# Xharlie/BtcDet

Hardware: AMD Instinct MI355X
Metric: scenes/s fwd+bwd KITTI-Car bs=2/GPU (BtcDet hot path) (higher is better)
Workload: dtype f32

## Files before the change

btcdet_amd/csrc/btc_common.h:

```cpp
#pragma once
#include <hip/hip_runtime.h>
#include <stdint.h>
#include <stdio.h>

#include "../../include/btcdet_hip.h"

#define BTC_EMPTY_KEY (-1)
#define BTC_EMPTY_IDX 0x7F7F7F7F

void btc_set_error(const char* fmt, ...);

#define BTC_CHECK_ARG(cond, ...)            \
  do {                                      \
    if (!(cond)) {                          \
      btc_set_error(__VA_ARGS__);           \
      return BTC_EINVAL;                    \
    }                                       \
  } while (0)

#define BTC_HIP(call)                                                             \
  do {                                                                            \
    hipError_t e_ = (call);                                                       \
    if (e_ != hipSuccess) {                                                       \
      btc_set_error("%s failed: %s (%s:%d)", #call, hipGetErrorString(e_), __FILE__, __LINE__); \
      return BTC_ELAUNCH;                                                         \
    }                                                                             \
  } while (0)

#define BTC_LAUNCH_CHECK()                                                        \
  do {                                                                            \
    hipError_t e_ = hipGetLastError();                                            \
    if (e_ != hipSuccess) {                                                       \
      btc_set_error("kernel launch failed: %s (%s:%d)", hipGetErrorString(e_), __FILE__, __LINE__); \
      return BTC_ELAUNCH;                                                         \
    }                                                                             \
  } while (0)

#if defined(__HIP_DEVICE_COMPILE__) && !defined(__gfx950__)
#error "the fence-free last-arriver protocol (btc_ticket_take) is derived for gfx950's sc1 write-through stores only"
#endif
#if defined(__HIPCC__)
template <class T>
__device__ __forceinline__ void btc_st_agent(T* p, T v) { __hip_atomic_store(p, v, __ATOMIC_RELAXED, __HIP_MEMORY_SCOPE_AGENT); }
template <class T>
__device__ __forceinline__ T btc_ld_agent(const T* p) { return __hip_atomic_load(p, __ATOMIC_RELAXED, __HIP_MEMORY_SCOPE_AGENT); }
__device__ __forceinline__ int btc_ticket_take(int32_t* counter) {
  asm volatile("s_waitcnt vmcnt(0)" ::: "memory");
  return __hip_atomic_fetch_add(counter, 1, __ATOMIC_RELAXED, __HIP_MEMORY_SCOPE_AGENT);
}
__device__ __forceinline__ void btc_ticket_acquire() { __builtin_amdgcn_fence(__ATOMIC_ACQUIRE, "agent"); }
#endif

#define BTC_TUNE_KEYS 24
int btc_tune_get(int key);

bool btc_apply_glds_supported(int K, int Cred, int Cres);
bool btc_apply_glds_has_shape(int shape, bool bf = false);
size_t btc_apply_glds_lds_bytes(int shape, int kc, int K, bool bf, int stages = 3);
int btc_apply_glds_stages(int shape, int kc, int K, bool bf, int asked);
int btc_launch_apply_glds(bool trans_w, int shape, int kc, int xcd, bool bf, const void* feat, const float* W, const float* bias,
                          const int32_t* nbr, const int32_t* order , int n_rows, int K, int Cred, int Cres, void* out,
                          hipStream_t stream, const struct BnFuse* bn = nullptr );

int btc_apply(const char* who, int pass, int operands, const void* src, long long src_rows, const void* W, const float* bias, const int32_t* nbr,
              const int32_t* order, int n_rows, int K, int Cin, int Cout, void* dst, hipStream_t stream, const struct BnFuse* bn);

int btc_apply_bf16w(const void* src, const void* Wq, const float* bias, const int32_t* nbr, const int32_t* order, int n_rows, int K, int Cred,
                    int Cres, void* dst, hipStream_t stream, int mirror = 0, const struct BnFuse* bn = nullptr);
constexpr size_t BTC_SCRATCH_HEAD = 64 * 1024;
constexpr long long BTC_SCRATCH_TICKETS = BTC_SCRATCH_HEAD / 4;
void* btc_scratch(hipStream_t stream, size_t* bytes);
struct BnFuse;
int btc_apply_split(const float* src, const void* Ws, const float* bias, const int32_t* nbr, const int32_t* order, int n_rows, int K, int Cred,
                    int Cres, float* dst, hipStream_t stream, int mirror, const BnFuse* bn);

__host__ __device__ __forceinline__ unsigned short btc_f32_to_bf16(float f) {
  union { float f; unsigned u; } c;
  c.f = f;
  unsigned u = c.u;
  if ((u & 0x7fffffffu) > 0x7f800000u) return (unsigned short)((u >> 16) | 0x40);
  u += 0x7fffu + ((u >> 16) & 1u);
  return (unsigned short)(u >> 16);
}
__host__ __device__ __forceinline__ float btc_bf16_to_f32(unsigned short h) {
  union { float f; unsigned u; } c;
  c.u = (unsigned)h << 16;
  return c.f;
}

template <bool BF>
__device__ __forceinline__ float4 btc_ld4(const float* base, size_t i) {
  if (!BF) return *reinterpret_cast<const float4*>(base + i);
  const uint2 v = *reinterpret_cast<const uint2*>(reinterpret_cast<const unsigned short*>(base) + i);
  return make_float4(__uint_as_float(v.x << 16), __uint_as_float(v.x & 0xffff0000u), __uint_as_float(v.y << 16),
                     __uint_as_float(v.y & 0xffff0000u));
}
template <bool BF>
__device__ __forceinline__ float btc_ld1(const float* base, size_t i) {
  if (!BF) return base[i];
  return __uint_as_float((unsigned)reinterpret_cast<const unsigned short*>(base)[i] << 16);
}
template <bool BF>
__device__ __forceinline__ void btc_st4(float* base, size_t i, float a, float b, float c, float d) {
  if (!BF) {
    *reinterpret_cast<float4*>(base + i) = make_float4(a, b, c, d);
  } else {
    uint2 v;
    v.x = (unsigned)btc_f32_to_bf16(a) | ((unsigned)btc_f32_to_bf16(b) << 16);
    v.y = (unsigned)btc_f32_to_bf16(c) | ((unsigned)btc_f32_to_bf16(d) << 16);
    *reinterpret_cast<uint2*>(reinterpret_cast<unsigned short*>(base) + i) = v;
  }
}
template <bool BF>
__device__ __forceinline__ void btc_st1(float* base, size_t i, float a) {
  if (!BF) base[i] = a;
  else reinterpret_cast<unsigned short*>(base)[i] = btc_f32_to_bf16(a);
}

#ifdef __cplusplus
#include <mutex>
constexpr int BTC_MAX_DEVICES = 16;
struct BtcPerDeviceOnce {
  std::once_flag flag[BTC_MAX_DEVICES];
};
template <class F>
static inline void btc_once_per_device(BtcPerDeviceOnce& o, F&& fn) {
  int dev = 0;
  (void)hipGetDevice(&dev);
  std::call_once(o.flag[dev >= 0 && dev < BTC_MAX_DEVICES ? dev : 0], fn);
}
#endif

typedef float f32x4 __attribute__((ext_vector_type(4)));
constexpr int TM = 64;
__host__ __device__ constexpr int ldb_of(int nt) { return nt * 16 + (((nt * 16) % 32 == 0) ? 16 : 0); }

static inline int btc_cdiv(long long a, long long b) { return (int)((a + b - 1) / b); }
static inline size_t btc_align(size_t x, size_t a = 256) { return (x + a - 1) / a * a; }
static inline unsigned btc_pow2_ge(unsigned long long v) {
  unsigned long long p = 1;
  while (p < v) p <<= 1;
  return (unsigned)p;
}

struct BtcCarver {
  char* base;
  size_t off;
  explicit BtcCarver(void* p) : base((char*)p), off(0) {}
  template <typename T>
  T* take(size_t count) {
    T* r = (T*)(base + off);
    off += btc_align(count * sizeof(T));
    return r;
  }
};

size_t btc_scan_ws_bytes(long long n);
int btc_scan_exclusive_i32(const int32_t* in, int32_t* out, long long n, int32_t* total, void* ws, hipStream_t stream);

size_t btc_bytemap_bytes(long long nwords);
int btc_bytemap_to_ranked_bitmap(const unsigned char* bytemap, long long nwords, unsigned* bitmap, int32_t* prefix, int32_t* total,
                                 void* ws, hipStream_t stream);

struct BtcGeom {
  int in_shape[3];
  int out_shape[3];
  int k[3];
  int s[3];
  int p[3];
  int d[3];
  int K;
  int mode;
};

__device__ __forceinline__ unsigned btc_hash32(unsigned key) {
  key *= 2654435761u;
  key ^= key >> 15;
  return key;
}
```

btcdet_amd/csrc/conv_apply_bf16.hip:

```cpp
#include "conv_tile.h"

namespace {

__device__ unsigned short g_zero_row_b[128];

constexpr int B_STAGES = 3;

template <int WR, int WC, int NTW, int KC, bool PAIR = false>
__global__ __launch_bounds__(64 * WR * WC) void conv_apply_b(const unsigned short* __restrict__ feat, const unsigned short* __restrict__ Wq,
                                                             const float* __restrict__ bias, const int32_t* __restrict__ nbr,
                                                             const int32_t* __restrict__ order, int n_rows, int K, int Cred, int Cres,
                                                             unsigned short* __restrict__ out, int flags, const BnFuse bn) {
  extern __shared__ __attribute__((aligned(16))) char smem[];
  constexpr int NW = WR * WC, THREADS = 64 * NW;
  constexpr int TM = 16 * WR, TN = 16 * NTW * WC;
  constexpr int UPR = KC / 8;
  constexpr int RPB = (128 / (KC * 2)) < 1 ? 1 : (128 / (KC * 2));
  constexpr int A_UNITS = TM * UPR, B_UNITS = TN * UPR;
  constexpr int NAI_TOTAL = (A_UNITS + 63) / 64, NAI = (NAI_TOTAL + NW - 1) / NW;
  constexpr int NBI_TOTAL = (B_UNITS + 63) / 64, NBI = (NBI_TOTAL + NW - 1) / NW;
  constexpr int NPI = NAI + NBI;
  constexpr int A_BYTES = (TM * KC * 2 + 1023) / 1024 * 1024;
  constexpr int B_BYTES = (TN * KC * 2 + 1023) / 1024 * 1024;
  constexpr int STAGE = A_BYTES + B_BYTES;
  char* ring = smem;
  APPLY_TAIL(ring + B_STAGES * STAGE, TM, K);

  const int tid = threadIdx.x, lane = tid & 63, wave = tid >> 6;
  const int wr = wave / WC, wc = wave % WC;
  const ApplyTile tile = apply_tile_prologue<TM, THREADS>(s_nbr, s_kact, s_nact, s_row, nbr, order, n_rows, K, flags, wr);
  const int bx = tile.bx, n0 = blockIdx.y * TN, n_act = tile.n_act;
  const unsigned long long wave_act = tile.wave_act;
  static_assert(!PAIR || KC == 64, "PAIR: two 32-channel offsets per 64-channel item");
  const int n_chunks = PAIR ? 1 : Cred / KC;
  const int n_items = PAIR ? (n_act + 1) >> 1 : n_act * n_chunks;

  f32x4 acc[NTW];
#pragma unroll
  for (int nt = 0; nt < NTW; ++nt) acc[nt] = (f32x4){0.f, 0.f, 0.f, 0.f};

  int iq = 0, ir = 0, cq = 0, cr = 0;
  auto issue = [&](int st) {
    const int k = s_kact[PAIR ? 2 * iq : iq];
    const int k1 = (PAIR && 2 * iq + 1 < n_act) ? s_kact[2 * iq + 1] : -1;
    const int cc = PAIR ? 0 : ir * KC;
    if (++ir == n_chunks) { ir = 0; ++iq; }
    char* As = ring + st * STAGE;
    char* Bs = As + A_BYTES;
#pragma unroll
    for (int t = 0; t < NAI; ++t) {
      const int ai = (wave + NW * t) % NAI_TOTAL;
      const int U = ai * 64 + lane;
      if (A_UNITS % 64 == 0 || U < A_UNITS) {
        const int rloc = U / UPR;
        const int u = (U % UPR) ^ ((rloc / RPB) & (UPR - 1));
        const int ku = (PAIR && (u & 4)) ? k1 : k;
        const int nb = ku >= 0 ? s_nbr[rloc * K + ku] : -1;
        const unsigned short* src = nb >= 0 ? feat + (size_t)nb * Cred + cc + (PAIR ? (u & 3) : u) * 8 : g_zero_row_b;
        glds16(src, As + ai * 1024);
      }
    }
    const unsigned short* Wk = Wq + ((size_t)k * Cres + n0) * Cred + cc;
    const unsigned short* Wk1 = PAIR ? Wq + ((size_t)(k1 >= 0 ? k1 : k) * Cres + n0) * Cred : Wk;
#pragma unroll
    for (int t = 0; t < NBI; ++t) {
      const int bi = (wave + NW * t) % NBI_TOTAL;
      const int U = bi * 64 + lane;
      if (B_UNITS % 64 == 0 || U < B_UNITS) {
        const int c = U / UPR;
        const int u = (U % UPR) ^ ((c / RPB) & (UPR - 1));
        glds16(((PAIR && (u & 4)) ? Wk1 : Wk) + (size_t)c * Cred + (PAIR ? (u & 3) : u) * 8, Bs + bi * 1024);
      }
    }
  };

  const int arow = lane & 15, kq = lane >> 4;
  if (n_items > 0) issue(0);
  if (n_items > 1) issue(1);
  int st = 0;
  for (int item = 0; item < n_items; ++item) {
    if (item + 1 < n_items) wait_vm<NPI>();
    else wait_vm<0>();
    __builtin_amdgcn_s_barrier();
    asm volatile("" ::: "memory");
    if (item + 2 < n_items) issue(st == 0 ? 2 : st - 1);
    const int k = s_kact[PAIR ? 2 * cq : cq];
    const int k2 = (PAIR && 2 * cq + 1 < n_act) ? s_kact[2 * cq + 1] : -1;
    if (++cr == n_chunks) { cr = 0; ++cq; }
    const bool act0 = (wave_act >> k) & 1ull, act1 = PAIR && k2 >= 0 && ((wave_act >> k2) & 1ull);
    if (act0 || act1) {
      const char* A = ring + st * STAGE + (wr * 16 + arow) * (KC * 2);
      const char* B = ring + st * STAGE + A_BYTES;
      const int aswz = ((wr * 16 + arow) / RPB) & (UPR - 1);
      constexpr int STEPS = KC / 32;
      bf16x8 a[STEPS], b[STEPS][NTW];
#pragma unroll
      for (int s = 0; s < STEPS; ++s) {
        const int q = s * 4 + kq;
        a[s] = *(const bf16x8*)(A + ((q ^ aswz) * 16));
#pragma unroll
        for (int nt = 0; nt < NTW; ++nt) {
          const int col = (wc * NTW + nt) * 16 + arow;
          b[s][nt] = *(const bf16x8*)(B + col * (KC * 2) + ((q ^ ((col / RPB) & (UPR - 1))) * 16));
        }
      }
#pragma unroll
      for (int s = 0; s < STEPS; ++s) {
        if (PAIR && !(s ? act1 : act0)) continue;
#pragma unroll
        for (int nt = 0; nt < NTW; ++nt)
          acc[nt] = __builtin_amdgcn_mfma_f32_16x16x32_bf16(a[s], b[s][nt], acc[nt], 0, 0, 0);
      }
    }
    st = (st == B_STAGES - 1) ? 0 : st + 1;
  }

  float vals[NTW][4];
  bool valid[4];
  int rows[4];
#pragma unroll
  for (int r = 0; r < 4; ++r) rows[r] = s_row[wr * 16 + kq * 4 + r];
  apply_tile_epilogue<NTW>(acc, rows, n0 + wc * NTW * 16, bias, Cres, out, bn, bn.ev_mean != nullptr, vals, valid);
  if (bn.slots) {
    bn_fuse_wave<NTW>(bn, vals, valid, n0 + wc * NTW * 16, (int)((bx * WR + wr) & (bn.nslots - 1)));
    bn_fuse_finish(bn, (int*)smem, (double*)(smem + 16));
  }
}

size_t lds_bytes_b(int tm, int tn, int kc, int K) {
  const size_t a = ((size_t)tm * kc * 2 + 1023) / 1024 * 1024, b = ((size_t)tn * kc * 2 + 1023) / 1024 * 1024;
  return (size_t)B_STAGES * (a + b) + apply_tail_bytes(tm, K);
}

template <int WR, int WC, int NTW, int KC, bool PAIR = false>
int launch_b(const unsigned short* feat, const unsigned short* Wq, const float* bias, const int32_t* nbr, const int32_t* order, int n_rows, int K, int Cred,
             int Cres, unsigned short* out, int flags, hipStream_t stream, const BnFuse& bn) {
  constexpr int TM = 16 * WR, TN = 16 * NTW * WC;
  return apply_launch<conv_apply_b<WR, WC, NTW, KC, PAIR>>("conv_apply_b", dim3(btc_cdiv(n_rows, TM), Cres / TN), 64 * WR * WC, lds_bytes_b(TM, TN, KC, K),
                                                          stream, feat, Wq, bias, nbr, order, n_rows, K, Cred, Cres, out, flags, bn);
}

template <int WR, int WC, int NTW>
int launch_b_kc(int kc, const unsigned short* feat, const unsigned short* Wq, const float* bias, const int32_t* nbr, const int32_t* order, int n_rows,
                int K, int Cred, int Cres, unsigned short* out, int xcd, hipStream_t stream, const BnFuse& bn) {
  if (kc == 128) return launch_b<WR, WC, NTW, 64, true>(feat, Wq, bias, nbr, order, n_rows, K, Cred, Cres, out, xcd, stream, bn);
  if (kc == 64) return launch_b<WR, WC, NTW, 64>(feat, Wq, bias, nbr, order, n_rows, K, Cred, Cres, out, xcd, stream, bn);
  return launch_b<WR, WC, NTW, 32>(feat, Wq, bias, nbr, order, n_rows, K, Cred, Cres, out, xcd, stream, bn);
}

int apply_b(const void* feat_, const void* Wq_, const float* bias, const int32_t* nbr, const int32_t* order, int n_rows, int K, int Cred, int Cres,
            void* out_, hipStream_t stream, int mirror = 0, const BnFuse* bn_ = nullptr) {
  if (n_rows <= 0) return BTC_OK;
  const BnFuse bn = bn_ ? *bn_ : btc_bn_fuse_none();
  const unsigned short* feat = (const unsigned short*)feat_;
  const unsigned short* Wq = (const unsigned short*)Wq_;
  unsigned short* out = (unsigned short*)out_;
  int kc = (Cred % 64 == 0) ? 64 : 32;
  if (Cred == 32 && K >= 8 && btc_tune_get(BTC_TUNE_SPLIT_PAIR) != 1 && (btc_tune_get(BTC_TUNE_SPLIT_PAIR) == 2 || n_rows >= 5000)) kc = 128;
  const int xcd = apply_flags(mirror);
  if (Cres % 128 == 0) return launch_b_kc<4, 2, 4>(kc, feat, Wq, bias, nbr, order, n_rows, K, Cred, Cres, out, xcd, stream, bn);
  if (Cres % 64 == 0) {
    if (n_rows < 8192) return launch_b_kc<1, 4, 1>(kc, feat, Wq, bias, nbr, order, n_rows, K, Cred, Cres, out, xcd, stream, bn);
    return launch_b_kc<4, 2, 2>(kc, feat, Wq, bias, nbr, order, n_rows, K, Cred, Cres, out, xcd, stream, bn);
  }
  if (Cres % 32 == 0) return launch_b_kc<2, 2, 1>(kc, feat, Wq, bias, nbr, order, n_rows, K, Cred, Cres, out, xcd, stream, bn);
  return launch_b_kc<4, 1, 1>(kc, feat, Wq, bias, nbr, order, n_rows, K, Cred, Cres, out, xcd, stream, bn);
}

constexpr int BF16_MULTI_MAX = 32;
struct Bf16Table {
  const float* W[BF16_MULTI_MAX];
  unsigned short* w_b[BF16_MULTI_MAX];
  unsigned short* wt_b[BF16_MULTI_MAX];
  int K[BF16_MULTI_MAX], Cin[BF16_MULTI_MAX], Cout[BF16_MULTI_MAX], first_block[BF16_MULTI_MAX + 1];
  int n;
};

__global__ __launch_bounds__(256) void weights_to_bf16_multi(const Bf16Table t) {
  int s = 0;
  while (s + 1 < t.n && (int)blockIdx.x >= t.first_block[s + 1]) ++s;
  const long long e = (long long)((int)blockIdx.x - t.first_block[s]) * 256 + threadIdx.x;
  const int Cin = t.Cin[s], Cout = t.Cout[s];
  const long long per = (long long)Cin * Cout;
  if (e >= (long long)t.K[s] * per) return;
  const unsigned short h = btc_f32_to_bf16(t.W[s][e]);
  t.w_b[s][e] = h;
  const int k = (int)(e / per);
  const int rem = (int)(e - (long long)k * per);
  const int ci = rem / Cout, co = rem - ci * Cout;
  t.wt_b[s][(long long)k * per + (long long)co * Cin + ci] = h;
}

}

extern "C" int btc_weights_to_bf16_multi(const float* const* W, void* const* w_bf16, void* const* wt_bf16, const int32_t* K, const int32_t* Cin,
                                         const int32_t* Cout, int n, void* stream) {
  BTC_CHECK_ARG(n >= 0, "btc_weights_to_bf16_multi: bad count");
  for (int base = 0; base < n; base += BF16_MULTI_MAX) {
    Bf16Table t;
    t.n = n - base < BF16_MULTI_MAX ? n - base : BF16_MULTI_MAX;
    int blocks = 0;
    for (int i = 0; i < t.n; ++i) {
      BTC_CHECK_ARG(K[base + i] >= 1 && Cin[base + i] >= 1 && Cout[base + i] >= 1, "btc_weights_to_bf16_multi: bad sizes");
      t.W[i] = W[base + i];
      t.w_b[i] = (unsigned short*)w_bf16[base + i];
      t.wt_b[i] = (unsigned short*)wt_bf16[base + i];
      t.K[i] = K[base + i]; t.Cin[i] = Cin[base + i]; t.Cout[i] = Cout[base + i];
      t.first_block[i] = blocks;
      blocks += (int)btc_cdiv((long long)K[base + i] * Cin[base + i] * Cout[base + i], 256);
    }
    t.first_block[t.n] = blocks;
    if (blocks > 0) weights_to_bf16_multi<<<blocks, 256, 0, (hipStream_t)stream>>>(t);
    BTC_LAUNCH_CHECK();
  }
  return BTC_OK;
}

int btc_apply_bf16w(const void* src, const void* Wq, const float* bias, const int32_t* nbr, const int32_t* order, int n_rows, int K, int Cred,
                    int Cres, void* dst, hipStream_t stream, int mirror, const BnFuse* bn) {
  return apply_b(src, Wq, bias, nbr, order, n_rows, K, Cred, Cres, dst, stream, mirror, bn);
}

extern "C" int btc_conv_bf16w_supported(int K, int Cred, int Cres) { return K >= 1 && K <= 64 && Cred >= 32 && Cred % 32 == 0 && Cres % 16 == 0; }

extern "C" int btc_weights_to_bf16(const float* W, int K, int Cin, int Cout, void* w_bf16, void* wt_bf16, void* stream) {
  BTC_CHECK_ARG(K >= 1 && Cin >= 1 && Cout >= 1, "btc_weights_to_bf16: bad sizes");
  return btc_weights_to_bf16_multi(&W, &w_bf16, &wt_bf16, &K, &Cin, &Cout, 1, stream);
}
```

btcdet_amd/csrc/conv_apply_glds.hip:

```cpp
#include "conv_tile.h"

namespace {

__device__ float g_zero_row[64];

constexpr int G_STAGES_DEFAULT = 3;
constexpr int G_STAGES_MAX = 8;

__device__ __forceinline__ void transpose4(const f32x4 v, float& y0, float& y1, float& y2, float& y3) {
  unsigned x0 = __float_as_uint(v[0]), x1 = __float_as_uint(v[1]), x2 = __float_as_uint(v[2]), x3 = __float_as_uint(v[3]);
  auto a = __builtin_amdgcn_permlane32_swap(x0, x2, false, false);
  x0 = a[0]; x2 = a[1];
  auto b = __builtin_amdgcn_permlane32_swap(x1, x3, false, false);
  x1 = b[0]; x3 = b[1];
  auto c = __builtin_amdgcn_permlane16_swap(x0, x1, false, false);
  x0 = c[0]; x1 = c[1];
  auto d = __builtin_amdgcn_permlane16_swap(x2, x3, false, false);
  x2 = d[0]; x3 = d[1];
  y0 = __uint_as_float(x0); y1 = __uint_as_float(x1); y2 = __uint_as_float(x2); y3 = __uint_as_float(x3);
}

template <int WR, int WC, int NTW, bool TRANS_W, int KC, bool BF>
__global__ __launch_bounds__(64 * WR * WC) void conv_apply_g(const void* __restrict__ feat_, const float* __restrict__ W,
                                                             const float* __restrict__ bias, const int32_t* __restrict__ nbr,
                                                             const int32_t* __restrict__ order, int n_rows, int K, int Cred, int Cres,
                                                             void* __restrict__ out_, int flags, int dbg, const BnFuse bn) {
  extern __shared__ __attribute__((aligned(16))) char smem[];
  const int S = ((flags >> APPLY_STAGES_SHIFT) & 15) ? ((flags >> APPLY_STAGES_SHIFT) & 15) : G_STAGES_DEFAULT;
  constexpr int NW = WR * WC, THREADS = 64 * NW;
  constexpr int TM = 16 * WR, TN = 16 * NTW * WC, NG = NTW * WC;
  constexpr int ES = BF ? 2 : 4;
  constexpr int UPR = KC * ES / 16;
  constexpr int UPB = KC / 4;
  constexpr int RPB = (128 / (KC * ES)) < 1 ? 1 : (128 / (KC * ES));
  constexpr int A_UNITS = TM * UPR;
  constexpr int NAI_TOTAL = (A_UNITS + 63) / 64;
  constexpr int NAI = (NAI_TOTAL + NW - 1) / NW;
  constexpr int NBI_TOTAL = KC * TN / 256;
  constexpr int NBI = (NBI_TOTAL + NW - 1) / NW;
  constexpr int NPI = NAI + NBI;
  constexpr int A_BYTES = (TM * KC * ES + 1023) / 1024 * 1024;
  constexpr int STAGE = A_BYTES + KC * TN * 4;
  char* ring = smem;
  APPLY_TAIL(ring + S * STAGE, TM, K);
  const char* feat = (const char*)feat_;

  const int tid = threadIdx.x, lane = tid & 63, wave = tid >> 6;
  const int wr = wave / WC, wc = wave % WC;
  const ApplyTile tile = apply_tile_prologue<TM, THREADS>(s_nbr, s_kact, s_nact, s_row, nbr, order, n_rows, K, flags, wr);
  const int bx = tile.bx, n0 = blockIdx.y * TN, n_act = tile.n_act;
  const unsigned long long wave_act = tile.wave_act;
  const int n_chunks = Cred / KC;
  const int n_items = (dbg & 32) ? 0 : n_act * n_chunks;
  if (dbg & 16) return;

  f32x4 acc[NTW];
#pragma unroll
  for (int nt = 0; nt < NTW; ++nt) acc[nt] = (f32x4){0.f, 0.f, 0.f, 0.f};

  int iq = 0, ir = 0, cq = 0, cr = 0;
  auto issue = [&](int st) {
    const int k = s_kact[iq];
    const int cc = ir * KC;
    if (++ir == n_chunks) { ir = 0; ++iq; }
    char* As = ring + st * STAGE;
    float* Bs = (float*)(As + A_BYTES);
#pragma unroll
    for (int t = 0; t < NAI; ++t) {
      if (dbg & 8) break;
      const int ai = (wave + NW * t) % NAI_TOTAL;
      const int U = ai * 64 + lane;
      if (A_UNITS % 64 == 0 || U < A_UNITS) {
        const int rloc = U / UPR;
        const int u = (U % UPR) ^ ((rloc / RPB) & (UPR - 1));
        const int nb = s_nbr[rloc * K + k];
        const char* src = nb >= 0 ? feat + ((size_t)nb * Cred + cc) * ES + u * 16 : (const char*)g_zero_row;
        glds16(src, As + ai * 1024);
      }
    }
    const float* Wk = W + (size_t)k * Cred * Cres;
#pragma unroll
    for (int t = 0; t < NBI; ++t) {
      if (dbg & 4) break;
      const int ii = (wave + NW * t) % NBI_TOTAL;
      const int U = ii * 64 + lane;
      const float* src;
      if (!TRANS_W) {
        const int kr = U / (TN / 4), pu = U % (TN / 4);
        const int g = (NG >= 2) ? ((pu >> 2) ^ (kr & 1)) : (pu >> 2);
        src = Wk + (size_t)(cc + kr) * Cres + n0 + g * 16 + (pu & 3) * 4;
      } else {
        const int c = U / UPB, pu = U % UPB;
        const int ru = pu ^ (c & (UPB - 1));
        src = Wk + (size_t)(n0 + c) * Cred + cc + ru * 4;
      }
      glds16(src, Bs + ii * 256);
    }
  };

  const int arow = lane & 15, kq = lane >> 4;
#define WAIT_ITEMS(n) wait_vm<((n) * NPI > 63 ? 63 : (n) * NPI)>()
  for (int i = 0; i < S - 1 && i < n_items; ++i) issue(i);
  int st = 0;
  for (int item = 0; item < n_items; ++item) {
    const int left = n_items - 1 - item, fl = left < S - 2 ? left : S - 2;
    switch (fl) {
      case 0: wait_vm<0>(); break;
      case 1: WAIT_ITEMS(1); break;
      case 2: WAIT_ITEMS(2); break;
      case 3: WAIT_ITEMS(3); break;
      case 4: WAIT_ITEMS(4); break;
      case 5: WAIT_ITEMS(5); break;
      default: WAIT_ITEMS(6); break;
    }
#undef WAIT_ITEMS
    __builtin_amdgcn_s_barrier();
    asm volatile("" ::: "memory");
    if (item + S - 1 < n_items && !(dbg & 2)) issue(st == 0 ? S - 1 : st - 1);
    const int k = s_kact[cq];
    if (++cr == n_chunks) { cr = 0; ++cq; }
    if (((wave_act >> k) & 1ull) && !(dbg & 1)) {
      const char* A = ring + st * STAGE + (wr * 16 + arow) * (KC * ES);
      const float* B = (const float*)(ring + st * STAGE + A_BYTES);
      const int aswz = ((wr * 16 + arow) / RPB) & (UPR - 1);
      constexpr int Q = KC / 4;
      constexpr int G = (16 / NTW) < 1 ? 1 : ((16 / NTW) > Q ? Q : (16 / NTW));
      constexpr int NGRP = Q / G;
      float a[2][G], b[2][G][NTW];
      constexpr bool A128 = !BF && (G % 4 == 0);
      constexpr bool B128 = TRANS_W && (G % 4 == 0) && UPB >= 8 && NTW == 1;
      auto load_group = [&](int g, int buf) {
        if (A128) {
#pragma unroll
          for (int jb = 0; jb < G / 4; ++jb) {
            const int u = (g * (G / 4) + jb) * 4 + kq;
            const f32x4 v = *(const f32x4*)(A + ((u ^ aswz) * 16));
            transpose4(v, a[buf][4 * jb], a[buf][4 * jb + 1], a[buf][4 * jb + 2], a[buf][4 * jb + 3]);
          }
        }
        if (B128) {
#pragma unroll
          for (int nt = 0; nt < NTW; ++nt) {
            const float* colp = B + ((wc * NTW + nt) * 16 + arow) * KC;
#pragma unroll
            for (int jb = 0; jb < G / 4; ++jb) {
              const int u = (g * (G / 4) + jb) * 4 + kq;
              const f32x4 v = *(const f32x4*)(colp + ((u ^ (arow & (UPB - 1))) * 4));
              transpose4(v, b[buf][4 * jb][nt], b[buf][4 * jb + 1][nt], b[buf][4 * jb + 2][nt], b[buf][4 * jb + 3][nt]);
            }
          }
        }
#pragma unroll
        for (int i = 0; i < G; ++i) {
          const int q = g * G + i;
          if (A128) {
          } else if (!BF) {
            a[buf][i] = *(const float*)(A + ((q ^ aswz) * 16) + kq * 4);
          } else {
            const unsigned short h = *(const unsigned short*)(A + (((q >> 1) ^ aswz) * 16) + (((q & 1) * 4 + kq) * 2));
            a[buf][i] = __uint_as_float((unsigned)h << 16);
          }
          if (!TRANS_W) {
            const float* bp = B + (q * 4 + kq) * TN + arow;
#pragma unroll
            for (int nt = 0; nt < NTW; ++nt) {
              const int cg = wc * NTW + nt;
              b[buf][i][nt] = bp[((NG >= 2) ? (cg ^ (kq & 1)) : cg) * 16];
            }
          } else if (!B128) {
            const float* bp = B + (wc * NTW * 16 + arow) * KC + (q ^ (arow & (UPB - 1))) * 4 + kq;
#pragma unroll
            for (int nt = 0; nt < NTW; ++nt) b[buf][i][nt] = bp[nt * 16 * KC];
          }
        }
      };
      load_group(0, 0);
#pragma unroll
      for (int g = 0; g < NGRP; ++g) {
        if (g + 1 < NGRP) load_group(g + 1, (g + 1) & 1);
        __builtin_amdgcn_sched_barrier(0);
#pragma unroll
        for (int i = 0; i < G; ++i)
#pragma unroll
          for (int nt = 0; nt < NTW; ++nt)
            acc[nt] = __builtin_amdgcn_mfma_f32_16x16x4f32(a[g & 1][i], b[g & 1][i][nt], acc[nt], 0, 0, 0);
        __builtin_amdgcn_sched_barrier(0);
      }
    }
    st = (st == S - 1) ? 0 : st + 1;
  }

  float vals[NTW][4];
  bool valid[4];
  int rows[4];
#pragma unroll
  for (int r = 0; r < 4; ++r) rows[r] = s_row[wr * 16 + kq * 4 + r];
  const bool ev = !TRANS_W && bn.ev_mean != nullptr;
  typedef typename std::conditional<BF, unsigned short, float>::type OUT;
  apply_tile_epilogue<NTW>(acc, rows, n0 + wc * NTW * 16, bias, Cres, (OUT*)out_, bn, ev, vals, valid);
  if (bn.slots) {
    bn_fuse_wave<NTW>(bn, vals, valid, n0 + wc * NTW * 16, (int)((bx * WR + wr) & (bn.nslots - 1)));
    bn_fuse_finish(bn, (int*)smem, (double*)(smem + 16));
  }
}

template <int WR, int WC, int NTW, bool TRANS_W, int KC, bool BF>
int launch_g(const void* feat, const float* W, const float* bias, const int32_t* nbr, const int32_t* order, int n_rows, int K, int Cred,
             int Cres, void* out, int xcd, hipStream_t stream, const BnFuse& bn) {
  constexpr int TM = 16 * WR, TN = 16 * NTW * WC;
  const int stages = btc_apply_glds_stages(WR * 100 + WC * 10 + NTW, KC, K, BF, (xcd >> APPLY_STAGES_SHIFT) & 15);
  xcd = (xcd & (APPLY_XCD | APPLY_MIRROR)) | (stages << APPLY_STAGES_SHIFT);
  const size_t lds = btc_apply_glds_lds_bytes(WR * 100 + WC * 10 + NTW, KC, K, BF, stages);
  return apply_launch<conv_apply_g<WR, WC, NTW, TRANS_W, KC, BF>>("conv_apply_g", dim3(btc_cdiv(n_rows, TM), Cres / TN), 64 * WR * WC, lds, stream, feat, W,
                                                                  bias, nbr, order, n_rows, K, Cred, Cres, out, xcd,
                                                                  btc_tune_get(BTC_TUNE_APPLY_DEBUG), bn);
}

#define G_ARGS feat, W, bias, nbr, order, n_rows, K, Cred, Cres, out, xcd, stream, bn
#define G_PARAMS                                                                                                             \
  const void *feat, const float *W, const float *bias, const int32_t *nbr, const int32_t *order, int n_rows, int K, int Cred, int Cres, \
      void *out, int xcd, hipStream_t stream, const BnFuse &bn

template <int WR, int WC, int NTW, bool TRANS_W, bool BF>
int launch_g_kc(int kc, G_PARAMS) {
  switch (kc) {
    case 16: return launch_g<WR, WC, NTW, TRANS_W, 16, BF>(G_ARGS);
    case 32: return launch_g<WR, WC, NTW, TRANS_W, 32, BF>(G_ARGS);
    default: return launch_g<WR, WC, NTW, TRANS_W, 64, BF>(G_ARGS);
  }
}

template <bool TRANS_W>
int launch_g_shape(int wr, int wc, int ntw, int kc, bool bf, G_PARAMS) {
  const int code = wr * 100 + wc * 10 + ntw;
  switch (code) {
#define G_CASE2(WR_, WC_, NTW_)                                                      \
  case WR_ * 100 + WC_ * 10 + NTW_:                                                  \
    return bf ? launch_g_kc<WR_, WC_, NTW_, TRANS_W, true>(kc, G_ARGS) : launch_g_kc<WR_, WC_, NTW_, TRANS_W, false>(kc, G_ARGS)
#define G_CASE(WR_, WC_, NTW_)      \
  case WR_ * 100 + WC_ * 10 + NTW_: \
    if (bf) break;                  \
    return launch_g_kc<WR_, WC_, NTW_, TRANS_W, false>(kc, G_ARGS)
    G_CASE2(4, 1, 1); G_CASE(4, 1, 2); G_CASE(4, 1, 4); G_CASE(4, 1, 8);
    G_CASE(4, 2, 1); G_CASE2(4, 2, 2); G_CASE2(4, 2, 4);
    G_CASE2(2, 2, 1); G_CASE(2, 2, 2); G_CASE(2, 2, 4);
    G_CASE(2, 4, 1); G_CASE(2, 4, 2);
    G_CASE2(1, 4, 1); G_CASE(1, 4, 2);
#undef G_CASE
#undef G_CASE2
    default: break;
  }
  btc_set_error("conv_apply_g: no instance for WR=%d WC=%d NTW=%d bf16=%d", wr, wc, ntw, (int)bf);
  return BTC_EINVAL;
}

}

bool btc_apply_glds_has_shape(int shape, bool bf) {
  static const int shapes[] = {411, 412, 414, 418, 421, 422, 424, 221, 222, 224, 241, 242, 141, 142};
  static const int shapes_bf[] = {411, 422, 424, 221, 141};
  if (bf) {
    for (int v : shapes_bf)
      if (v == shape) return true;
    return false;
  }
  for (int v : shapes)
    if (v == shape) return true;
  return false;
}

size_t btc_apply_glds_lds_bytes(int shape, int kc, int K, bool bf, int stages) {
  const int tm = 16 * (shape / 100), tn = 16 * ((shape / 10) % 10) * (shape % 10);
  const size_t a_bytes = ((size_t)tm * kc * (bf ? 2 : 4) + 1023) / 1024 * 1024;
  return (size_t)(stages > 0 ? stages : G_STAGES_DEFAULT) * (a_bytes + (size_t)kc * tn * 4) + apply_tail_bytes(tm, K);
}

int btc_apply_glds_stages(int shape, int kc, int K, bool bf, int asked) {
  const int tm = 16 * (shape / 100), tn = 16 * ((shape / 10) % 10) * (shape % 10), nw = (shape / 100) * ((shape / 10) % 10);
  const size_t a_bytes = ((size_t)tm * kc * (bf ? 2 : 4) + 1023) / 1024 * 1024, stage = a_bytes + (size_t)kc * tn * 4;
  const int npi = (int)(((a_bytes / 1024) + nw - 1) / nw + ((size_t)kc * tn / 256 + nw - 1) / nw);
  int s = asked ? asked : btc_tune_get(BTC_TUNE_APPLY_STAGES);
  if (!s) {
    s = (int)((size_t)48 * 1024 / stage);
    if (s > 6) s = 6;
  }
  if (s < 3) s = 3;
  if (s > G_STAGES_MAX) s = G_STAGES_MAX;
  while (s > 3 && ((s - 2) * npi > 63 || btc_apply_glds_lds_bytes(shape, kc, K, bf, s) > 160 * 1024)) --s;
  return s;
}

bool btc_apply_glds_supported(int K, int Cred, int Cres) { return K <= 64 && Cred % 16 == 0 && Cres % 16 == 0 && Cred >= 16; }

int btc_launch_apply_glds(bool trans_w, int shape, int kc, int xcd, bool bf, const void* feat, const float* W, const float* bias,
                          const int32_t* nbr, const int32_t* order, int n_rows, int K, int Cred, int Cres, void* out, hipStream_t stream,
                          const BnFuse* bn_) {
  if (n_rows <= 0) return BTC_OK;
  const BnFuse bn = bn_ ? *bn_ : btc_bn_fuse_none();
  const int wr = shape / 100, wc = (shape / 10) % 10, ntw = shape % 10;
  BTC_CHECK_ARG(btc_apply_glds_supported(K, Cred, Cres) && wc * ntw > 0 && Cres % (16 * wc * ntw) == 0 && Cred % kc == 0 &&
                    (kc == 16 || kc == 32 || kc == 64),
                "conv_apply_g: unsupported K=%d Cred=%d Cres=%d shape=%d kc=%d", K, Cred, Cres, shape, kc);
  return trans_w ? launch_g_shape<true>(wr, wc, ntw, kc, bf, G_ARGS) : launch_g_shape<false>(wr, wc, ntw, kc, bf, G_ARGS);
}
```

btcdet_amd/csrc/conv_apply_split.hip:

```cpp
#include "conv_tile.h"

namespace {

#define BTC_RSRC_RECORDS 0xFFFFFF00u
#define BTC_RSRC_ABSENT 0xFFFFFFF0u
__device__ __forceinline__ void blds16s(__amdgpu_buffer_rsrc_t rsrc, unsigned voffset, void* l) {
  __builtin_amdgcn_raw_ptr_buffer_load_lds(rsrc, (__attribute__((address_space(3))) void*)l, 16, voffset, 0, 0, 0);
}

template <int WR, int WC, int NTW, int KC, int S_STAGES, int LW, bool PAIR = false>
__global__ __launch_bounds__(64 * (WR * WC + LW)) void conv_apply_s(const float* __restrict__ feat, const unsigned short* __restrict__ Ws,
                                                             const float* __restrict__ bias, const int32_t* __restrict__ nbr,
                                                             const int32_t* __restrict__ order, int n_rows, int K, int Cred, int Cres,
                                                             float* __restrict__ out, int flags, const BnFuse bn) {
  extern __shared__ __attribute__((aligned(16))) char smem[];
  constexpr int NW = WR * WC, THREADS = 64 * (NW + LW);
  constexpr int NLD = LW ? LW : NW;
  constexpr int TM = 16 * WR, TN = 16 * NTW * WC;
  constexpr int UPA = KC / 4, UPB = KC / 8;
  constexpr int A_UNITS = TM * UPA, B_UNITS = 3 * TN * UPB;
  static_assert(A_UNITS % 64 == 0 && B_UNITS % 64 == 0, "whole DMA instructions");
  constexpr int NAI_TOTAL = A_UNITS / 64, NAI = (NAI_TOTAL + NLD - 1) / NLD;
  constexpr int NBI_TOTAL = B_UNITS / 64, NBI = (NBI_TOTAL + NLD - 1) / NLD;
  static_assert(LW == 0 || (NAI_TOTAL % LW == 0 && NBI_TOTAL % LW == 0), "the loader waves share the pieces evenly");
  constexpr int NPI = NAI + NBI;
  constexpr int A_BYTES = TM * KC * 4, P_BYTES = TN * KC * 2;
  constexpr int STAGE = A_BYTES + 3 * P_BYTES;
  char* ring = smem;
  APPLY_TAIL(ring + S_STAGES * STAGE, TM, K);

  const int tid = threadIdx.x, lane = tid & 63, wave = tid >> 6;
  const bool computes = LW == 0 || wave < NW, loads = LW == 0 || wave >= NW;
  const int wr = computes ? wave / WC : 0, wc = wave % WC;
  const int lid = LW ? wave - NW : wave;
  const int dbg = flags >> APPLY_DEBUG_SHIFT;
  const ApplyTile tile = apply_tile_prologue<TM, THREADS>(s_nbr, s_kact, s_nact, s_row, nbr, order, n_rows, K, flags, wr);
  const int bx = tile.bx, n0 = blockIdx.y * TN;
  const unsigned long long wave_act = tile.wave_act;
  const size_t plane = (size_t)K * Cred * Cres;
  const int n_act = __builtin_amdgcn_readfirstlane(tile.n_act);
  static_assert(!PAIR || KC == 64, "PAIR: two 32-channel offsets per 64-channel item");
  const int n_chunks = PAIR ? 1 : Cred / KC;
  const int n_pairs = PAIR ? (n_act + 1) >> 1 : n_act;
  const int n_all = n_pairs * n_chunks;
  const int i0 = (int)((long long)blockIdx.z * n_all / gridDim.z);
  const int n_items = (dbg & 32) ? i0 : (int)((long long)(blockIdx.z + 1) * n_all / gridDim.z);
  out += (size_t)blockIdx.z * n_rows * Cres;

  int iq = i0 / n_chunks, ir = i0 - iq * n_chunks;
  int cq = iq, cr = ir;
  const __amdgpu_buffer_rsrc_t rfeat = __builtin_amdgcn_make_buffer_rsrc((void*)feat, 0, BTC_RSRC_RECORDS, 0x00020000);
  const int kvec = lane < n_act ? s_kact[lane] : 0;
  int nbq[NAI];
  auto load_nbq = [&]() {
    if (PAIR) {
      const int k0 = __builtin_amdgcn_readlane(kvec, (2 * iq) & 63);
      const int k1 = (2 * iq + 1 < n_act) ? __builtin_amdgcn_readlane(kvec, (2 * iq + 1) & 63) : -1;
#pragma unroll
      for (int t = 0; t < NAI; ++t) {
        const int U = ((lid + NLD * t) % NAI_TOTAL) * 64 + lane;
        const int rloc = U / UPA;
        const int u = (U % UPA) ^ ((rloc ^ (rloc >> 3)) & (UPA - 1));
        const int k = (u & 8) ? k1 : k0;
        nbq[t] = k >= 0 ? s_nbr[rloc * K + k] : -1;
      }
      return;
    }
    const int k = __builtin_amdgcn_readlane(kvec, iq);
#pragma unroll
    for (int t = 0; t < NAI; ++t) {
      const int U = ((lid + NLD * t) % NAI_TOTAL) * 64 + lane;
      nbq[t] = s_nbr[(U / UPA) * K + k];
    }
  };
  if (loads) load_nbq();
  const __amdgpu_buffer_rsrc_t rw = __builtin_amdgcn_make_buffer_rsrc((void*)Ws, 0, BTC_RSRC_RECORDS, 0x00020000);
  static_assert(NLD % 2 == 0 && (TN * UPB) % 64 == 0 && 64 % UPB == 0, "one lane offset per issuing wave");
  const int w_c = lane / UPB;
  const int w_su = (lane % UPB) ^ (((w_c >> 1) + (UPB == 8 ? 4 * (lid & 1) : 0)) & (UPB - 1));
  const unsigned w_lane = (unsigned)(w_c * Cred + (PAIR ? (w_su & 3) : w_su) * 8) * 2u;
  auto issue = [&](int st) {
    const int k = __builtin_amdgcn_readlane(kvec, PAIR ? ((2 * iq) & 63) : iq);
    const int k1 = PAIR ? ((2 * iq + 1 < n_act) ? __builtin_amdgcn_readlane(kvec, (2 * iq + 1) & 63) : k) : k;
    const unsigned w_lane_i = PAIR ? w_lane + ((w_su & 4) ? (unsigned)((size_t)(k1 - k) * Cres * Cred) * 2u : 0u) : w_lane;
    const int cc = ir * KC;
    char* As = ring + st * STAGE;
    char* Bs = As + A_BYTES;
#pragma unroll
    for (int t = 0; t < NAI; ++t) {
      if (dbg & 8) break;
      const int ai = (lid + NLD * t) % NAI_TOTAL;
      const int U = ai * 64 + lane;
      const int rloc = U / UPA;
      const int u = (U % UPA) ^ ((rloc ^ (rloc >> 3)) & (UPA - 1));
      const int nb = nbq[t];
      blds16s(rfeat, nb >= 0 ? ((unsigned)nb * (unsigned)Cred + (unsigned)(PAIR ? (u & 7) * 4 : cc + u * 4)) * 4u : BTC_RSRC_ABSENT, As + ai * 1024);
    }
    const unsigned w_item = (unsigned)(((size_t)k * Cres + n0) * Cred + (PAIR ? 0 : cc)) * 2u;
#pragma unroll
    for (int t = 0; t < NBI; ++t) {
      if (dbg & 4) break;
      const int bi = (lid + NLD * t) % NBI_TOTAL;
      const int pl = (bi * 64) / (TN * UPB), c0 = ((bi * 64) % (TN * UPB)) / UPB;
      const unsigned w_piece = (unsigned)((size_t)pl * plane + (size_t)c0 * Cred) * 2u;
      __builtin_amdgcn_raw_ptr_buffer_load_lds(rw, (__attribute__((address_space(3))) void*)(Bs + bi * 1024), 16, w_lane_i, w_item + w_piece, 0, 0);
    }
    if (++ir == n_chunks) {
      ir = 0;
      ++iq;
      load_nbq();
    }
  };

  const int arow = lane & 15, kg = lane >> 4;
  static_assert((S_STAGES - 2) * NPI <= 63, "vmcnt is a 6-bit counter");
  float vals[NTW][4];
  bool valid[4];
  if (LW > 0 && wave >= NW) {
#pragma unroll
    for (int i = 0; i < S_STAGES - 1; ++i)
      if (i0 + i < n_items) issue(i);
    int st = 0;
    for (int item = i0; item < n_items; ++item) {
      const int left = n_items - 1 - item;
      if (S_STAGES >= 4 && left >= 2) wait_vm<(S_STAGES >= 4 ? 2 : 0) * NPI>();
      else if (S_STAGES >= 3 && left >= 1) wait_vm<(S_STAGES >= 3 ? 1 : 0) * NPI>();
      else wait_vm<0>();
      __builtin_amdgcn_s_barrier();
      asm volatile("" ::: "memory");
      if (item + S_STAGES - 1 < n_items && !(dbg & 2)) issue(st == 0 ? S_STAGES - 1 : st - 1);
      st = (st == S_STAGES - 1) ? 0 : st + 1;
    }
#pragma unroll
    for (int nt = 0; nt < NTW; ++nt)
#pragma unroll
      for (int r = 0; r < 4; ++r) vals[nt][r] = 0.f;
#pragma unroll
    for (int r = 0; r < 4; ++r) valid[r] = false;
  } else {
    f32x4 acc[NTW], accm[NTW], accs[NTW];
#pragma unroll
    for (int nt = 0; nt < NTW; ++nt) acc[nt] = accm[nt] = accs[nt] = (f32x4){0.f, 0.f, 0.f, 0.f};
#pragma unroll
    for (int i = 0; i < S_STAGES - 1; ++i)
      if (LW == 0 && i0 + i < n_items) issue(i);
    int st = 0;
    for (int item = i0; item < n_items; ++item) {
      const int left = n_items - 1 - item;
      if (LW == 0) {
        if (S_STAGES >= 4 && left >= 2) wait_vm<(S_STAGES >= 4 ? 2 : 0) * NPI>();
        else if (S_STAGES >= 3 && left >= 1) wait_vm<(S_STAGES >= 3 ? 1 : 0) * NPI>();
        else wait_vm<0>();
      }
      __builtin_amdgcn_s_barrier();
      asm volatile("" ::: "memory");
      if (LW == 0 && item + S_STAGES - 1 < n_items && !(dbg & 2)) issue(st == 0 ? S_STAGES - 1 : st - 1);
      asm volatile("" ::: "memory");
      const int k = __builtin_amdgcn_readlane(kvec, PAIR ? ((2 * cq) & 63) : cq);
      const int k2 = (PAIR && 2 * cq + 1 < n_act) ? __builtin_amdgcn_readlane(kvec, (2 * cq + 1) & 63) : -1;
      if (++cr == n_chunks) { cr = 0; ++cq; }
      const bool act0 = (wave_act >> k) & 1ull, act1 = PAIR && k2 >= 0 && ((wave_act >> k2) & 1ull);
      if ((act0 || act1) && !(dbg & 1)) {
        const int r = wr * 16 + arow;
        const char* A = ring + st * STAGE + r * (KC * 4);
        const char* B = ring + st * STAGE + A_BYTES;
        const int aswz = (r ^ (r >> 3)) & (UPA - 1);
        constexpr int STEPS = KC / 32;
        constexpr int GS = (NTW >= 4) ? 1 : STEPS;
#pragma unroll
        for (int g = 0; g < STEPS / GS; ++g) {
          f32x4 av[GS][2];
          bf16x8 bh[GS][NTW], bm[GS][NTW], bl[GS][NTW];
#pragma unroll
          for (int j = 0; j < GS; ++j) {
            const int u0 = 8 * (g * GS + j) + 2 * kg;
            av[j][0] = *(const f32x4*)(A + ((u0 ^ aswz) * 16));
            av[j][1] = *(const f32x4*)(A + (((u0 + 1) ^ aswz) * 16));
          }
#pragma unroll
          for (int j = 0; j < GS; ++j)
#pragma unroll
            for (int nt = 0; nt < NTW; ++nt) {
              const int col = (wc * NTW + nt) * 16 + arow;
              const char* bp = B + col * (KC * 2) + (((4 * (g * GS + j) + kg) ^ ((col >> 1) & (UPB - 1))) * 16);
              bh[j][nt] = *(const bf16x8*)bp;
              bm[j][nt] = *(const bf16x8*)(bp + P_BYTES);
              bl[j][nt] = *(const bf16x8*)(bp + 2 * P_BYTES);
            }
          __builtin_amdgcn_sched_barrier(0);
#pragma unroll
          for (int j = 0; j < GS; ++j) {
            if (PAIR && !((g * GS + j) ? act1 : act0)) continue;
            const f32x4 v0 = av[j][0], v1 = av[j][1];
            uint4 ah, am, al;
            btc_split3(v0[0], v0[1], ah.x, am.x, al.x);
            btc_split3(v0[2], v0[3], ah.y, am.y, al.y);
            btc_split3(v1[0], v1[1], ah.z, am.z, al.z);
            btc_split3(v1[2], v1[3], ah.w, am.w, al.w);
            const bf16x8 Ah = __builtin_bit_cast(bf16x8, ah), Am = __builtin_bit_cast(bf16x8, am), Al = __builtin_bit_cast(bf16x8, al);
#define S_MFMA(ACC, X, Y)                 \
    _Pragma("unroll") for (int nt = 0; nt < NTW; ++nt) ACC[nt] = __builtin_amdgcn_mfma_f32_16x16x32_bf16(X, Y[j][nt], ACC[nt], 0, 0, 0)
            S_MFMA(accs, Al, bh);
            S_MFMA(accs, Ah, bl);
            S_MFMA(accs, Am, bm);
            S_MFMA(accm, Am, bh);
            S_MFMA(accm, Ah, bm);
            S_MFMA(acc, Ah, bh);
#undef S_MFMA
          }
        }
      }
      st = (st == S_STAGES - 1) ? 0 : st + 1;
    }

    const bool ev = bn.ev_mean != nullptr;
#pragma unroll
    for (int nt = 0; nt < NTW; ++nt) {
      const int col = n0 + (wc * NTW + nt) * 16 + (lane & 15);
      const float bv0 = bias ? bias[col] : 0.f;
      BnEvalCol ec = {0.f, 0.f, 1.f, 0.f};
      if (ev) ec = bn_eval_col(bn, col);
#pragma unroll
      for (int r = 0; r < 4; ++r) {
        const int row = s_row[wr * 16 + kg * 4 + r];
        valid[r] = row >= 0;
        const float sum = acc[nt][r] + (accm[nt][r] + accs[nt][r]);
        float v = bias ? (sum + bv0) : sum;
        if (ev) v = bn_affine(v, ec.m, ec.rs, ec.g, ec.b, bn.ev_relu);
        if (row >= 0) out[(size_t)row * Cres + col] = v;
        vals[nt][r] = v;
      }
    }
  }
  if (bn.slots) {
    if (computes) bn_fuse_wave<NTW>(bn, vals, valid, n0 + wc * NTW * 16, (int)((bx * WR + wr) & (bn.nslots - 1)));
    bn_fuse_finish(bn, (int*)smem, (double*)(smem + 16));
  }
}

size_t lds_bytes_s(int tm, int tn, int kc, int K, int stages) {
  return (size_t)stages * ((size_t)tm * kc * 4 + (size_t)3 * tn * kc * 2) + apply_tail_bytes(tm, K);
}

template <int WR, int WC, int NTW, int KC, int S_STAGES, int LW = 0, bool PAIR = false>
int launch_s(const float* feat, const unsigned short* Ws, const float* bias, const int32_t* nbr, const int32_t* order, int n_rows, int K, int Cred,
             int Cres, float* out, int flags, hipStream_t stream, const BnFuse& bn, int zsplit) {
  constexpr int TM = 16 * WR, TN = 16 * NTW * WC;
  return apply_launch<conv_apply_s<WR, WC, NTW, KC, S_STAGES, LW, PAIR>>("conv_apply_s", dim3(btc_cdiv(n_rows, TM), Cres / TN, zsplit), 64 * (WR * WC + LW),
                                                                        lds_bytes_s(TM, TN, KC, K, S_STAGES), stream, feat, Ws, bias, nbr, order, n_rows, K,
                                                                        Cred, Cres, out, flags, bn);
}

__global__ __launch_bounds__(256) void split_reduce(const float* __restrict__ slabs, int Z, const float* __restrict__ bias, int n_rows, int Cres,
                                                    float* __restrict__ out, const BnFuse bn) {
  __shared__ int s_flag;
  const int lane = threadIdx.x & 63, wave = threadIdx.x >> 6;
  const int cq = lane & 15, rq = lane >> 4;
  const int col = blockIdx.y * 64 + cq * 4;
  const int row0 = (blockIdx.x * 4 + wave) * 16;
  const size_t slab = (size_t)n_rows * Cres;
  const f32x4 b = bias ? *(const f32x4*)(bias + col) : (f32x4){0.f, 0.f, 0.f, 0.f};
  double s1[4] = {0.0, 0.0, 0.0, 0.0}, s2[4] = {0.0, 0.0, 0.0, 0.0};
  const bool ev = bn.ev_mean != nullptr;
  BnEvalCol ec[4] = {};
  if (ev) {
#pragma unroll
    for (int e = 0; e < 4; ++e) ec[e] = bn_eval_col(bn, col + e);
  }
#pragma unroll
  for (int i = 0; i < 4; ++i) {
    const int row = row0 + i * 4 + rq;
    if (row < n_rows) {
      const float* p = slabs + (size_t)row * Cres + col;
      f32x4 v = *(const f32x4*)p;
      for (int z = 1; z < Z; ++z) v += *(const f32x4*)(p + z * slab);
      if (bias) v += b;
      if (ev) {
#pragma unroll
        for (int e = 0; e < 4; ++e) v[e] = bn_affine(v[e], ec[e].m, ec[e].rs, ec[e].g, ec[e].b, bn.ev_relu);
      }
      *(f32x4*)(out + (size_t)row * Cres + col) = v;
#pragma unroll
      for (int e = 0; e < 4; ++e) {
        s1[e] += (double)v[e];
        s2[e] += (double)v[e] * (double)v[e];
      }
    }
  }
  if (bn.slots) {
    const int slot = (int)((blockIdx.x * 4 + wave) & (bn.nslots - 1));
#pragma unroll
    for (int e = 0; e < 4; ++e) {
      s1[e] += __shfl_xor(s1[e], 16, 64);
      s2[e] += __shfl_xor(s2[e], 16, 64);
      s1[e] += __shfl_xor(s1[e], 32, 64);
      s2[e] += __shfl_xor(s2[e], 32, 64);
      if (lane < 16 && col + e < bn.C) {
        double* p = bn.slots + ((size_t)slot * 2) * BN_FUSE_CMAX + col + e;
        unsafeAtomicAdd(p, s1[e]);
        unsafeAtomicAdd(p + BN_FUSE_CMAX, s2[e]);
      }
    }
    bn_fuse_finish(bn, &s_flag);
  }
}

constexpr int SPLIT_MULTI_MAX = 32;
struct SplitTable {
  const float* W[SPLIT_MULTI_MAX];
  unsigned short* w_s[SPLIT_MULTI_MAX];
  unsigned short* wt_s[SPLIT_MULTI_MAX];
  int K[SPLIT_MULTI_MAX], Cin[SPLIT_MULTI_MAX], Cout[SPLIT_MULTI_MAX], first_block[SPLIT_MULTI_MAX + 1];
  int n;
};

__global__ __launch_bounds__(256) void weights_split3_multi(const SplitTable t) {
  int s = 0;
  while (s + 1 < t.n && (int)blockIdx.x >= t.first_block[s + 1]) ++s;
  const long long e = (long long)((int)blockIdx.x - t.first_block[s]) * 256 + threadIdx.x;
  const int Cin = t.Cin[s], Cout = t.Cout[s];
  const long long per = (long long)Cin * Cout, n = (long long)t.K[s] * per;
  if (e >= n) return;
  const BtcSplit3 x = btc_split3(t.W[s][e]);
  const unsigned short p[3] = {(unsigned short)(x.hi >> 16), (unsigned short)(x.mid >> 16), (unsigned short)(x.lo >> 16)};
  const int k = (int)(e / per);
  const int rem = (int)(e - (long long)k * per);
  const int ci = rem / Cout, co = rem - ci * Cout;
  const long long et = (long long)k * per + (long long)co * Cin + ci;
#pragma unroll
  for (int j = 0; j < 3; ++j) {
    t.w_s[s][j * n + e] = p[j];
    t.wt_s[s][j * n + et] = p[j];
  }
}

}

extern "C" int btc_weights_split3_multi(const float* const* W, void* const* w_split, void* const* wt_split, const int32_t* K, const int32_t* Cin,
                                        const int32_t* Cout, int n, void* stream) {
  BTC_CHECK_ARG(n >= 0, "btc_weights_split3_multi: bad count");
  for (int base = 0; base < n; base += SPLIT_MULTI_MAX) {
    SplitTable t;
    t.n = n - base < SPLIT_MULTI_MAX ? n - base : SPLIT_MULTI_MAX;
    int blocks = 0;
    for (int i = 0; i < t.n; ++i) {
      BTC_CHECK_ARG(K[base + i] >= 1 && Cin[base + i] >= 1 && Cout[base + i] >= 1, "btc_weights_split3_multi: bad sizes");
      t.W[i] = W[base + i];
      t.w_s[i] = (unsigned short*)w_split[base + i];
      t.wt_s[i] = (unsigned short*)wt_split[base + i];
      t.K[i] = K[base + i]; t.Cin[i] = Cin[base + i]; t.Cout[i] = Cout[base + i];
      t.first_block[i] = blocks;
      blocks += (int)btc_cdiv((long long)K[base + i] * Cin[base + i] * Cout[base + i], 256);
    }
    t.first_block[t.n] = blocks;
    if (blocks > 0) weights_split3_multi<<<blocks, 256, 0, (hipStream_t)stream>>>(t);
    BTC_LAUNCH_CHECK();
  }
  return BTC_OK;
}

extern "C" int btc_conv_split_supported(int K, int Cred, int Cres) {
  return K >= 1 && K <= 64 && Cred >= 32 && Cred % 32 == 0 && Cres >= 32 && Cres % 32 == 0;
}

static bool btc_split_pair_wanted(int K, int n_rows, int shape) { return K >= 8 && shape != 422 && n_rows >= 5000; }

extern "C" int btc_conv_split_wanted(int K, int Cred, int Cres, int n_rows) {
  return btc_tune_get(BTC_TUNE_SPLIT) != 1 && btc_conv_split_supported(K, Cred, Cres) &&
         n_rows >= ((Cred >= 128 || Cres >= 128) ? 2500 : (Cres % 64 == 0 ? (Cred >= 64 ? 2500 : 6000) : 20000));
}

int btc_apply_split(const float* src, const void* Ws_, const float* bias_, const int32_t* nbr, const int32_t* order, int n_rows, int K, int Cred,
                    int Cres, float* dst_, hipStream_t stream, int mirror, const BnFuse* bn_) {
  if (n_rows <= 0) return BTC_OK;
  const float* bias = bias_;
  float* dst = dst_;
  BTC_CHECK_ARG(btc_conv_split_supported(K, Cred, Cres), "conv_apply_s: needs K <= 64, Cred %% 32 == 0, Cres %% 64 == 0 (K=%d, %d -> %d)", K, Cred, Cres);
  const BnFuse bn = bn_ ? *bn_ : btc_bn_fuse_none();
  const unsigned short* Ws = (const unsigned short*)Ws_;
  const int flags = apply_flags(mirror) | (btc_tune_get(BTC_TUNE_APPLY_DEBUG) << APPLY_DEBUG_SHIFT);
  const int t_nt = btc_tune_get(BTC_TUNE_APPLY_NT);
  size_t scratch_bytes = 0;
  float* scratch = (float*)btc_scratch(stream, &scratch_bytes);
  const int t_z = btc_tune_get(BTC_TUNE_SPLIT_Z);
  const bool few = n_rows < 10000;
  if (scratch_bytes > BTC_SCRATCH_HEAD) {
    scratch = (float*)((char*)scratch + BTC_SCRATCH_HEAD);
    scratch_bytes -= BTC_SCRATCH_HEAD;
  } else {
    scratch = nullptr;
    scratch_bytes = 0;
  }
  const bool can_z = few && t_z != 1 && scratch_bytes >= (size_t)2 * n_rows * Cres * sizeof(float);
  int shape = (Cres % 128 == 0) ? ((!few || can_z || Cres >= 256) ? 424 : 222) : ((!few || can_z) ? 422 : 222);
  if (Cres % 64 != 0) shape = n_rows >= 100000 ? 412 : 812;
  if ((Cres % 128 != 0 && n_rows >= 5000 && n_rows < 22000) || (K <= 4 && n_rows < 22000)) shape = 412;
  if (Cres % 64 != 0 && Cred == 32 && K >= 8 && n_rows >= 5000 && btc_tune_get(BTC_TUNE_SPLIT_PAIR) != 1 && btc_tune_get(BTC_TUNE_APPLY_KC) != 32) shape = 412;
  if ((t_nt == 812 || t_nt == 412) && Cres % 32 == 0) shape = t_nt;
  if ((t_nt == 224 || t_nt == 424) && Cres % 128 == 0) shape = t_nt;
  if ((t_nt == 222 || t_nt == 422 || t_nt == 414 || t_nt == 814) && Cres % 64 == 0) shape = t_nt;
  if ((t_nt == 418 || t_nt == 818) && Cres % 128 == 0) shape = t_nt;
  const int t_kc = btc_tune_get(BTC_TUNE_APPLY_KC), t_st = btc_tune_get(BTC_TUNE_APPLY_STAGES);
  int kc = (Cred % 64 == 0 && (shape % 10 == 4 || n_rows < 22000) && shape % 100 != 12) ? 64 : 32;
  if (t_kc == 32 || (t_kc == 64 && Cred % 64 == 0)) kc = t_kc;
  if (shape % 100 == 12) kc = (Cred % 64 == 0 && t_kc != 32) ? 64 : 32;
  if (shape == 818) kc = 32;
  const int t_pair = btc_tune_get(BTC_TUNE_SPLIT_PAIR);
  const bool pair = Cred == 32 && t_pair != 1 && t_kc != 32 && (shape == 412 || shape == 812 || shape == 422) && (t_pair == 2 || btc_split_pair_wanted(K, n_rows, shape));
  if (pair) kc = 64;
  int stages = t_st ? t_st : 3;
  if (kc == 64) stages = (t_st == 3 && shape == 422) ? 3 : 2;
  const int items = K * (Cred / kc);
  int Z = 1;
  if (can_z && shape % 100 != 12 && items >= 12) {
    Z = t_z > 1 ? t_z : ((Cres % 128 == 0 || n_rows < 4000) ? 4 : 2);
    if (Z > items / 6) Z = items / 6;
    while (Z > 1 && (size_t)Z * n_rows * Cres * sizeof(float) > scratch_bytes) --Z;
    if (Z > 1) dst = scratch;
  }
  const BnFuse bn_kernel = Z > 1 ? btc_bn_fuse_none() : bn;
  if (Z > 1) bias = nullptr;
#define S_ARGS src, Ws, bias, nbr, order, n_rows, K, Cred, Cres, dst, flags, stream, bn_kernel, Z
  int rc = BTC_EINVAL;
  const int t_lw = btc_tune_get(BTC_TUNE_SPLIT_LOADERS);
  int lw = t_lw == 2 ? 2 : (t_lw == 4 ? 4 : (t_lw == 1 ? 0 : (kc == 64 ? 4 : (shape == 412 ? 2 : 0))));
  {
    const int tm = (shape / 100) * 16, tn = 16 * ((shape / 10) % 10) * (shape % 10);
    if (lw == 4 && ((tm * kc / 256) % 4 != 0 || (3 * tn * kc / 512) % 4 != 0)) lw = 2;
  }
#define S_CASE(code, WR_, WC_, NTW_, KC_, ST_)                                                                          \
  case code:                                                                                                           \
    if constexpr ((16 * WR_ * KC_ / 256) % 4 == 0 && (3 * 16 * NTW_ * WC_ * KC_ / 512) % 4 == 0) {                       \
      if (lw == 4) { rc = launch_s<WR_, WC_, NTW_, KC_, ST_, 4>(S_ARGS); break; }                                       \
    }                                                                                                                  \
    rc = lw ? launch_s<WR_, WC_, NTW_, KC_, ST_, 2>(S_ARGS) : launch_s<WR_, WC_, NTW_, KC_, ST_, 0>(S_ARGS);            \
    break
#define S_PAIR(code, WR_, WC_, NTW_)                                                                                     \
  case code:                                                                                                           \
    rc = lw == 4 ? launch_s<WR_, WC_, NTW_, 64, 2, 4, true>(S_ARGS)                                                      \
                 : (lw ? launch_s<WR_, WC_, NTW_, 64, 2, 2, true>(S_ARGS) : launch_s<WR_, WC_, NTW_, 64, 2, 0, true>(S_ARGS)); \
    break
  if (pair) {
    switch (shape) {
      S_PAIR(412, 4, 1, 2);
      S_PAIR(812, 8, 1, 2);
      S_PAIR(422, 4, 2, 2);
    }
#undef S_PAIR
    return rc;
  }
  switch (shape * 10 + stages + (kc == 64 ? 5 : 0)) {
    S_CASE(4243, 4, 2, 4, 32, 3);
    S_CASE(4244, 4, 2, 4, 32, 4);
    S_CASE(4247, 4, 2, 4, 64, 2);
    S_CASE(2243, 2, 2, 4, 32, 3);
    S_CASE(2247, 2, 2, 4, 64, 2);
    S_CASE(2227, 2, 2, 2, 64, 2);
    S_CASE(4228, 4, 2, 2, 64, 3);
    S_CASE(2244, 2, 2, 4, 32, 4);
    S_CASE(4223, 4, 2, 2, 32, 3);
    S_CASE(4224, 4, 2, 2, 32, 4);
    S_CASE(4227, 4, 2, 2, 64, 2);
    S_CASE(4127, 4, 1, 2, 64, 2);
    S_CASE(8127, 8, 1, 2, 64, 2);
    S_CASE(4123, 4, 1, 2, 32, 3);
    S_CASE(4124, 4, 1, 2, 32, 4);
    S_CASE(8123, 8, 1, 2, 32, 3);
    S_CASE(8124, 8, 1, 2, 32, 4);
    S_CASE(4147, 4, 1, 4, 64, 2);
    S_CASE(4143, 4, 1, 4, 32, 3);
    S_CASE(8147, 8, 1, 4, 64, 2);
    S_CASE(8143, 8, 1, 4, 32, 3);
    S_CASE(4187, 4, 1, 8, 64, 2);
    S_CASE(4183, 4, 1, 8, 32, 3);
    case 8183: rc = launch_s<8, 1, 8, 32, 3, 0>(S_ARGS); break;
    S_CASE(2223, 2, 2, 2, 32, 3);
    S_CASE(2224, 2, 2, 2, 32, 4);
    default:
      btc_set_error("conv_apply_s: no instance for shape %d, %d stages, kc %d", shape, stages, kc);
      return BTC_EINVAL;
  }
#undef S_CASE
#undef S_ARGS
  if (rc != BTC_OK || Z == 1) return rc;
  split_reduce<<<dim3(btc_cdiv(n_rows, 64), Cres / 64), 256, 0, stream>>>(dst, Z, bias_, n_rows, Cres, dst_, bn);
  BTC_LAUNCH_CHECK();
  return BTC_OK;
}

extern "C" int btc_weights_split3(const float* W, int K, int Cin, int Cout, void* w_split, void* wt_split, void* stream) {
  BTC_CHECK_ARG(K >= 1 && Cin >= 1 && Cout >= 1, "btc_weights_split3: bad sizes");
  return btc_weights_split3_multi(&W, &w_split, &wt_split, &K, &Cin, &Cout, 1, stream);
}
```

btcdet_amd/csrc/conv_tile.h:

```cpp
#pragma once
#include <type_traits>

#include "btc_common.h"
#include "bn_fuse.h"

typedef __bf16 bf16x8 __attribute__((ext_vector_type(8)));

constexpr int APPLY_XCD = 1;
constexpr int APPLY_MIRROR = 2;
constexpr int APPLY_STAGES_SHIFT = 4;
constexpr int APPLY_DEBUG_SHIFT = 8;
inline int apply_flags(int mirror) { return (btc_tune_get(BTC_TUNE_APPLY_XCD) == 2 ? APPLY_XCD : 0) | (mirror ? APPLY_MIRROR : 0); }

inline size_t apply_tail_bytes(int tm, int K) { return (size_t)(tm * K + K + 1 + tm) * sizeof(int32_t); }
#define APPLY_TAIL(base, TM_, K_)              \
  int32_t* s_nbr = (int32_t*)(base);           \
  int32_t* s_kact = s_nbr + (TM_) * (K_);      \
  int32_t* s_nact = s_kact + (K_);             \
  int32_t* s_row = s_nact + 1

struct ApplyTile {
  int bx, row0, n_act;
  unsigned long long wave_act;
};

template <int TM, int THREADS>
__device__ __forceinline__ ApplyTile apply_tile_prologue(int32_t* s_nbr, int32_t* s_kact, int32_t* s_nact, int32_t* s_row, const int32_t* __restrict__ nbr,
                                                         const int32_t* __restrict__ order, int n_rows, int K, int flags, int wr) {
  const int tid = threadIdx.x, lane = tid & 63, wave = tid >> 6;
  const int mirror = (flags & APPLY_MIRROR) ? 1 : 0;
  int bx = blockIdx.x;
  if (flags & APPLY_XCD) {
    const int nb = gridDim.x, per = nb >> 3, main = per << 3;
    if (bx < main) bx = (bx & 7) * per + (bx >> 3);
  }
  const int row0 = bx * TM;
  for (int e = tid; e < K; e += THREADS) s_kact[e] = 0;
  for (int e = tid; e < TM; e += THREADS) s_row[e] = (row0 + e < n_rows) ? (order ? order[row0 + e] : row0 + e) : -1;
  __syncthreads();
  for (int e = tid; e < TM * K; e += THREADS) {
    const int rloc = e / K, kk = e - rloc * K;
    const int gr = s_row[rloc];
    const int v = gr >= 0 ? nbr[(long long)gr * K + (mirror ? K - 1 - kk : kk)] : -1;
    s_nbr[e] = v;
    if (v >= 0) s_kact[kk] = 1;
  }
  __syncthreads();
  unsigned long long wave_act;
  {
    bool any = false;
    if (lane < K)
      for (int r = 0; r < 16; ++r) any |= s_nbr[(wr * 16 + r) * K + lane] >= 0;
    wave_act = __ballot(any);
  }
  const int kflag = (lane < K) ? s_kact[lane] : 0;
  __syncthreads();
  if (wave == 0) {
    const unsigned long long m = __ballot(kflag != 0);
    if (kflag) s_kact[__popcll(m & ((1ull << lane) - 1ull))] = lane;
    if (lane == 0) *s_nact = __popcll(m);
  }
  __syncthreads();
  return {bx, row0, *s_nact, wave_act};
}

template <int NTW, bool COLS = false, typename OUT>
__device__ __forceinline__ void apply_tile_epilogue(const f32x4 (&sum)[NTW], const int (&rows)[4], int col0, const float* __restrict__ bias, int Cres,
                                                    OUT* __restrict__ out, const BnFuse& bn, bool ev, float (&vals)[NTW][4], bool (&valid)[4]) {
#pragma unroll
  for (int r = 0; r < 4; ++r) valid[r] = rows[r] >= 0;
#pragma unroll
  for (int nt = 0; nt < NTW; ++nt) {
    const int col = col0 + nt * 16 + (threadIdx.x & 15);
    const float bv0 = (bias && (!COLS || col < Cres)) ? bias[col] : 0.f;
    BnEvalCol ec = {0.f, 0.f, 1.f, 0.f};
    if (ev) ec = bn_eval_col(bn, col);
#pragma unroll
    for (int r = 0; r < 4; ++r) {
      float v = bias ? (sum[nt][r] + bv0) : sum[nt][r];
      if (sizeof(OUT) == 2) {
        unsigned short h = btc_f32_to_bf16(v);
        if (ev) h = btc_f32_to_bf16(bn_affine(btc_bf16_to_f32(h), ec.m, ec.rs, ec.g, ec.b, bn.ev_relu));
        if (rows[r] >= 0) ((unsigned short*)out)[(size_t)rows[r] * Cres + col] = h;
        v = btc_bf16_to_f32(h);
      } else {
        if (ev) v = bn_affine(v, ec.m, ec.rs, ec.g, ec.b, bn.ev_relu);
        if ((!COLS || col < Cres) && rows[r] >= 0) ((float*)out)[(size_t)rows[r] * Cres + col] = v;
      }
      vals[nt][r] = v;
    }
  }
}

__device__ __forceinline__ void glds16(const void* g, void* l) {
  __builtin_amdgcn_global_load_lds((const __attribute__((address_space(1))) void*)g, (__attribute__((address_space(3))) void*)l, 16, 0, 0);
}
template <int N>
__device__ __forceinline__ void wait_vm() {
  asm volatile("s_waitcnt vmcnt(%0)" ::"n"(N) : "memory");
}

__device__ __forceinline__ float btc_split_rest(float x) { return x - __uint_as_float(__float_as_uint(x) & 0xFFFF0000u); }
struct BtcSplit3 { unsigned hi, mid, lo; };
__device__ __forceinline__ BtcSplit3 btc_split3(float x) {
  const float x1 = btc_split_rest(x), x2 = btc_split_rest(x1);
  return {__float_as_uint(x), __float_as_uint(x1), __float_as_uint(x2)};
}
__device__ __forceinline__ void btc_split3(float a, float b, unsigned& hi, unsigned& mid, unsigned& lo) {
  hi = __builtin_amdgcn_perm(__float_as_uint(b), __float_as_uint(a), 0x07060302u);
  const float a1 = btc_split_rest(a), b1 = btc_split_rest(b);
  mid = __builtin_amdgcn_perm(__float_as_uint(b1), __float_as_uint(a1), 0x07060302u);
  const float a2 = btc_split_rest(a1), b2 = btc_split_rest(b1);
  lo = __builtin_amdgcn_perm(__float_as_uint(b2), __float_as_uint(a2), 0x07060302u);
}

constexpr size_t APPLY_LDS_MAX = 160 * 1024;
template <auto KERNEL, class... A>
int apply_launch(const char* who, dim3 grid, int threads, size_t lds, hipStream_t stream, A... args) {
  BTC_CHECK_ARG(lds <= APPLY_LDS_MAX, "%s: tile does not fit the LDS", who);
  static BtcPerDeviceOnce once;
  btc_once_per_device(once, [] { (void)hipFuncSetAttribute((const void*)KERNEL, hipFuncAttributeMaxDynamicSharedMemorySize, (int)APPLY_LDS_MAX); });
  hipLaunchKernelGGL(KERNEL, grid, dim3(threads), lds, stream, args...);
  BTC_LAUNCH_CHECK();
  return BTC_OK;
}
```

btcdet_amd/csrc/sparse_conv.hip:

```cpp
#include "conv_tile.h"

namespace {

constexpr int KC = 32;
constexpr int LDA = KC + 2;

template <int NT, bool TRANS_W, bool VEC, int KB, int THREADS>
__global__ __launch_bounds__(THREADS) void conv_apply(const float* __restrict__ feat, const float* __restrict__ W,
                                                  const float* __restrict__ bias, const int32_t* __restrict__ nbr,
                                                  int n_rows, int K, int Cred, int Cres, float* __restrict__ out, int mirror, const BnFuse bn) {
  extern __shared__ __attribute__((aligned(16))) char smem[];
  constexpr int TM = THREADS / 4;
  constexpr int LDB = ldb_of(NT);
  constexpr int NB = NT * 512 / THREADS;
  float* As = (float*)smem;
  float* Bs = As + KB * TM * LDA;
  int32_t* s_nbr = (int32_t*)(Bs + KB * KC * LDB);
  int32_t* s_kact = s_nbr + TM * K;
  int32_t* s_nact = s_kact + K;

  const int tid = threadIdx.x, lane = tid & 63, wave = tid >> 6;
  const int row0 = blockIdx.x * TM;
  const int n0 = blockIdx.y * (NT * 16);

  for (int e = tid; e < K; e += THREADS) s_kact[e] = 0;
  __syncthreads();
  {
    const long long gbase = (long long)row0 * K;
    const long long gend = (long long)n_rows * K;
    for (int e = tid; e < TM * K; e += THREADS) {
      const int kk = e % K;
      int v = (gbase + e < gend) ? nbr[mirror ? gbase + e - kk + (K - 1 - kk) : gbase + e] : -1;
      s_nbr[e] = v;
      if (v >= 0) s_kact[kk] = 1;
    }
  }
  __syncthreads();
  if (tid == 0) {
    int n = 0;
    for (int k = 0; k < K; ++k)
      if (s_kact[k]) s_kact[n++] = k;
    *s_nact = n;
  }
  __syncthreads();
  const int n_act = *s_nact;
  const int n_chunks = (KB > 1) ? 1 : (Cred + KC - 1) / KC;
  const int n_items = (KB > 1) ? (n_act + KB - 1) / KB : n_act * n_chunks;

  f32x4 acc[NT];
#pragma unroll
  for (int nt = 0; nt < NT; ++nt) acc[nt] = (f32x4){0.f, 0.f, 0.f, 0.f};
  const int arow = wave * 16 + (lane & 15);
  const int kq = lane >> 4;

  float4 av[KB][2];
  float as_[KB][8];
  float bv[KB][NB];

  int pq = 0, pr = 0, cr = 0;
  auto prefetch = [&](int item) {
    const int pq_now = pq, pr_now = pr;
    if (KB == 1 && ++pr == n_chunks) { pr = 0; ++pq; }
#pragma unroll
    for (int kb = 0; kb < KB; ++kb) {
      const int ai = (KB > 1) ? item * KB + kb : pq_now;
      const bool live = ai < n_act;
      const int k = live ? s_kact[ai] : 0;
      const int cc = (KB > 1) ? 0 : pr_now * KC;
      const int kc = min(KC, Cred - cc);
      const float* Wk = W + (size_t)k * Cred * Cres;
      if (VEC) {
#pragma unroll
        for (int i = 0; i < 2; ++i) {
          int e = i * THREADS + tid, r = e / (KC / 4), c = (e % (KC / 4)) * 4;
          int j = live ? s_nbr[r * K + k] : -1;
          av[kb][i] = (j >= 0 && c < kc) ? *reinterpret_cast<const float4*>(feat + (size_t)j * Cred + cc + c) : make_float4(0.f, 0.f, 0.f, 0.f);
        }
      } else {
#pragma unroll
        for (int i = 0; i < 8; ++i) {
          int e = i * THREADS + tid, r = e / KC, c = e % KC;
          int j = live ? s_nbr[r * K + k] : -1;
          as_[kb][i] = (j >= 0 && c < kc) ? feat[(size_t)j * Cred + cc + c] : 0.f;
        }
      }
#pragma unroll
      for (int i = 0; i < NB; ++i) {
        int e = i * THREADS + tid;
        if (!TRANS_W) {
          int r = e / (NT * 16), c = e % (NT * 16);
          bv[kb][i] = (live && r < kc && n0 + c < Cres) ? Wk[(size_t)(cc + r) * Cres + n0 + c] : 0.f;
        } else {
          int c = e / KC, r = e % KC;
          bv[kb][i] = (live && r < kc && n0 + c < Cres) ? Wk[(size_t)(n0 + c) * Cred + cc + r] : 0.f;
        }
      }
    }
  };
  auto commit = [&]() {
#pragma unroll
    for (int kb = 0; kb < KB; ++kb) {
      float* A = As + kb * TM * LDA;
      float* B = Bs + kb * KC * LDB;
      if (VEC) {
#pragma unroll
        for (int i = 0; i < 2; ++i) {
          int e = i * THREADS + tid, r = e / (KC / 4), c = (e % (KC / 4)) * 4;
          float* d = A + r * LDA + c;
          d[0] = av[kb][i].x; d[1] = av[kb][i].y; d[2] = av[kb][i].z; d[3] = av[kb][i].w;
        }
      } else {
#pragma unroll
        for (int i = 0; i < 8; ++i) {
          int e = i * THREADS + tid, r = e / KC, c = e % KC;
          A[r * LDA + c] = as_[kb][i];
        }
      }
#pragma unroll
      for (int i = 0; i < NB; ++i) {
        int e = i * THREADS + tid;
        if (!TRANS_W) {
          int r = e / (NT * 16), c = e % (NT * 16);
          B[r * LDB + c] = bv[kb][i];
        } else {
          int c = e / KC, r = e % KC;
          B[r * LDB + c] = bv[kb][i];
        }
      }
    }
  };

  if (n_items > 0) prefetch(0);
  for (int item = 0; item < n_items; ++item) {
    const int cc = (KB > 1) ? 0 : cr * KC;
    if (KB == 1 && ++cr == n_chunks) cr = 0;
    const int kc = min(KC, Cred - cc);
    __syncthreads();
    commit();
    __syncthreads();
    if (item + 1 < n_items) prefetch(item + 1);
    const int steps = (kc + 3) >> 2;
    const int cnt = (KB > 1) ? min(KB, n_act - item * KB) : 1;
#pragma unroll
    for (int kb = 0; kb < KB; ++kb) {
      if (kb >= cnt) break;
      const float* A = As + kb * TM * LDA;
      const float* B = Bs + kb * KC * LDB;
      for (int q = 0; q < steps; ++q) {
        float a = A[arow * LDA + q * 4 + kq];
        const float* bp = B + (q * 4 + kq) * LDB + (lane & 15);
#pragma unroll
        for (int nt = 0; nt < NT; ++nt) acc[nt] = __builtin_amdgcn_mfma_f32_16x16x4f32(a, bp[nt * 16], acc[nt], 0, 0, 0);
      }
    }
  }

  float vals[NT][4];
  bool valid[4];
  int rows[4];
#pragma unroll
  for (int r = 0; r < 4; ++r) rows[r] = row0 + wave * 16 + kq * 4 + r < n_rows ? row0 + wave * 16 + kq * 4 + r : -1;
  const bool ev = !TRANS_W && bn.ev_mean != nullptr;
  apply_tile_epilogue<NT, true>(acc, rows, n0, bias, Cres, out, bn, ev, vals, valid);
  if (bn.slots) {
    bn_fuse_wave<NT>(bn, vals, valid, n0, (int)((blockIdx.x * (THREADS / 64) + wave) & (bn.nslots - 1)));
    bn_fuse_finish(bn, (int*)smem, (double*)(smem + 16));
  }
}

constexpr int WS_WAVES = 16;
constexpr int WS_KB = 8;
constexpr int WS_Q = 2;

__host__ __device__ inline size_t ws_lds_bytes(int K, int Cred, int nt) {
  int crp = (Cred + 3) & ~3;
  return (size_t)K * crp * (nt * 16) * sizeof(float) + (size_t)WS_WAVES * 16 * K * sizeof(int32_t);
}

template <int NT, bool TRANS_W, bool EV = false>
__global__ __launch_bounds__(WS_WAVES * 64) void conv_apply_ws(const float* __restrict__ feat, const float* __restrict__ W,
                                                              const float* __restrict__ bias, const int32_t* __restrict__ nbr,
                                                              int n_rows, int K, int Cred, int Cres, float* __restrict__ out, int mirror,
                                                              const BnFuse bn) {
  extern __shared__ __attribute__((aligned(16))) char smem[];
  constexpr int LDW = NT * 16;
  constexpr int QMAX = WS_Q;
  const int crp = (Cred + 3) & ~3;
  float* Ws = (float*)smem;
  int32_t* nb_all = (int32_t*)(Ws + (size_t)K * crp * LDW);
  const int tid = threadIdx.x, lane = tid & 63, wave = tid >> 6, kq = lane >> 4, lrow = lane & 15;
  int32_t* nb = nb_all + wave * 16 * K;

  {
    const int total = K * crp * LDW;
    for (int base = 0; base < total; base += WS_WAVES * 64 * 8) {
      float v[8];
#pragma unroll
      for (int u = 0; u < 8; ++u) {
        int e = base + u * WS_WAVES * 64 + tid;
        int c = e % LDW, r = (e / LDW) % crp, k = e / (LDW * crp);
        v[u] = 0.f;
        if (e < total && r < Cred && c < Cres) v[u] = TRANS_W ? W[((size_t)k * Cres + c) * Cred + r] : W[((size_t)k * Cred + r) * Cres + c];
      }
#pragma unroll
      for (int u = 0; u < 8; ++u) {
        int e = base + u * WS_WAVES * 64 + tid;
        if (e < total) {
          int c = e % LDW, r = (e / LDW) % crp, k = e / (LDW * crp);
          int cs = (NT == 2) ? (c ^ ((r & 1) << 4)) : c;
          Ws[((size_t)k * crp + r) * LDW + cs] = v[u];
        }
      }
    }
  }
  __syncthreads();

  const int n_tiles = (n_rows + 15) >> 4;
  const int steps = crp >> 2;
  for (int tile = blockIdx.x * WS_WAVES + wave; tile < n_tiles; tile += gridDim.x * WS_WAVES) {
    const int row0 = tile << 4;
    unsigned long long kmask = 0;
    {
      const long long gbase = (long long)row0 * K, gend = (long long)n_rows * K;
      for (int e = lane; e < 16 * K; e += 64) {
        const int kk = e % K;
        int v = (gbase + e < gend) ? nbr[mirror ? gbase + e - kk + (K - 1 - kk) : gbase + e] : -1;
        nb[e] = v;
        if (v >= 0) kmask |= 1ull << kk;
      }
#pragma unroll
      for (int o = 32; o > 0; o >>= 1) kmask |= __shfl_xor(kmask, o, 64);
    }
    __builtin_amdgcn_wave_barrier();
    f32x4 acc[NT];
#pragma unroll
    for (int nt = 0; nt < NT; ++nt) acc[nt] = (f32x4){0.f, 0.f, 0.f, 0.f};

    float va[WS_KB][QMAX], vb[WS_KB][QMAX];
    int ka[WS_KB], kb_[WS_KB];
    unsigned long long rem = kmask;
#define WS_FETCH(v, kk)                                                                             \
  _Pragma("unroll") for (int g = 0; g < WS_KB; ++g) {                                               \
    kk[g] = rem ? (__ffsll((long long)rem) - 1) : -1;                                               \
    rem &= rem - 1;                                                                                 \
    const int j = (kk[g] >= 0) ? nb[lrow * K + kk[g]] : -1;                                         \
    const float* src = feat + (size_t)(j >= 0 ? j : 0) * Cred + kq;                                 \
    _Pragma("unroll") for (int q = 0; q < QMAX; ++q)                                                \
        v[g][q] = (j >= 0 && q * 4 + kq < Cred && q < steps) ? src[q * 4] : 0.f;                    \
  }
#define WS_MATH(v, kk)                                                                              \
  _Pragma("unroll") for (int g = 0; g < WS_KB; ++g) {                                               \
    if (kk[g] < 0) break;                                                                           \
    const float* Wk = Ws + (size_t)kk[g] * crp * LDW;                                               \
    _Pragma("unroll") for (int q = 0; q < QMAX; ++q) {                                              \
      if (q >= steps) break;                                                                        \
      const int r = q * 4 + kq;                                                                     \
      _Pragma("unroll") for (int nt = 0; nt < NT; ++nt) {                                           \
        int c = nt * 16 + lrow;                                                                     \
        if (NT == 2) c ^= (r & 1) << 4;                                                             \
        acc[nt] = __builtin_amdgcn_mfma_f32_16x16x4f32(v[g][q], Wk[r * LDW + c], acc[nt], 0, 0, 0); \
      }                                                                                             \
    }                                                                                               \
  }
    WS_FETCH(va, ka)
    while (ka[0] >= 0) {
      WS_FETCH(vb, kb_)
      WS_MATH(va, ka)
      if (kb_[0] < 0) break;
      WS_FETCH(va, ka)
      WS_MATH(vb, kb_)
    }
#undef WS_FETCH
#undef WS_MATH
    float vals[NT][4];
    bool valid[4];
    constexpr bool ev = EV;
#pragma unroll
    for (int r = 0; r < 4; ++r) valid[r] = row0 + kq * 4 + r < n_rows;
#pragma unroll
    for (int nt = 0; nt < NT; ++nt) {
      const int col = nt * 16 + lrow;
      const float bv0 = (bias && col < Cres) ? bias[col] : 0.f;
      BnEvalCol ec = {0.f, 0.f, 1.f, 0.f};
      if (ev) ec = bn_eval_col(bn, col);
#pragma unroll
      for (int r = 0; r < 4; ++r) {
        const int row = row0 + kq * 4 + r;
        vals[nt][r] = bias ? (acc[nt][r] + bv0) : acc[nt][r];
        if (ev) vals[nt][r] = bn_affine(vals[nt][r], ec.m, ec.rs, ec.g, ec.b, bn.ev_relu);
        if (col < Cres && row < n_rows) out[(size_t)row * Cres + col] = vals[nt][r];
      }
    }
    if (bn.slots) bn_fuse_wave<NT>(bn, vals, valid, 0, (int)(tile & (bn.nslots - 1)));
    __builtin_amdgcn_wave_barrier();
  }
  if (bn.slots) bn_fuse_finish(bn, (int*)smem, (double*)(smem + 16));
}


__global__ __launch_bounds__(256) void maxpool_fwd_k(const float* __restrict__ feat, const int32_t* __restrict__ nbr,
                                                     int n_out, int K, int C, float* __restrict__ out) {
  long long t = (long long)blockIdx.x * blockDim.x + threadIdx.x;
  if (t >= (long long)n_out * C) return;
  int i = (int)(t / C), c = (int)(t % C);
  float m = 0.f;
  for (int k = 0; k < K; ++k) {
    int j = nbr[(size_t)i * K + k];
    if (j >= 0) m = fmaxf(m, feat[(size_t)j * C + c]);
  }
  out[t] = m;
}

__global__ __launch_bounds__(256) void maxpool_bwd_k(const float* __restrict__ feat, const float* __restrict__ out,
                                                     const float* __restrict__ dout, const int32_t* __restrict__ nbr_in,
                                                     int n_in, int K, int C, float* __restrict__ din) {
  long long t = (long long)blockIdx.x * blockDim.x + threadIdx.x;
  if (t >= (long long)n_in * C) return;
  int j = (int)(t / C), c = (int)(t % C);
  float v = feat[t], g = 0.f;
  for (int k = 0; k < K; ++k) {
    int i = nbr_in[(size_t)j * K + k];
    if (i >= 0 && out[(size_t)i * C + c] == v) g += dout[(size_t)i * C + c];
  }
  din[t] = g;
}

__global__ __launch_bounds__(256) void dense_fwd_k(const float* __restrict__ feat, const int4* __restrict__ idx, int n, int C,
                                                   int D, int H, int Wd, float* __restrict__ dense) {
  long long t = (long long)blockIdx.x * blockDim.x + threadIdx.x;
  if (t >= (long long)n * C) return;
  int c = (int)(t / n), i = (int)(t % n);
  int4 q = idx[i];
  size_t vol = (size_t)D * H * Wd;
  dense[((size_t)q.x * C + c) * vol + ((size_t)q.y * H + q.z) * Wd + q.w] = feat[(size_t)i * C + c];
}

__global__ __launch_bounds__(256) void dense_bwd_k(const float* __restrict__ ddense, const int4* __restrict__ idx, int n, int C,
                                                   int D, int H, int Wd, float* __restrict__ dfeat) {
  long long t = (long long)blockIdx.x * blockDim.x + threadIdx.x;
  if (t >= (long long)n * C) return;
  int c = (int)(t / n), i = (int)(t % n);
  int4 q = idx[i];
  size_t vol = (size_t)D * H * Wd;
  dfeat[(size_t)i * C + c] = ddense[((size_t)q.x * C + c) * vol + ((size_t)q.y * H + q.z) * Wd + q.w];
}

template <int NT, bool TRANS_W, int THREADS>
int launch_apply_t(dim3 grid, size_t lds, hipStream_t stream, bool vec, const float* feat, const float* W, const float* bias,
                   const int32_t* nbr, int n_rows, int K, int Cred, int Cres, float* out, int mirror, const BnFuse& bn) {
  if (vec) return apply_launch<conv_apply<NT, TRANS_W, true, 1, THREADS>>("conv_apply", grid, THREADS, lds, stream, feat, W, bias, nbr, n_rows, K, Cred, Cres, out, mirror, bn);
  return apply_launch<conv_apply<NT, TRANS_W, false, 1, THREADS>>("conv_apply", grid, THREADS, lds, stream, feat, W, bias, nbr, n_rows, K, Cred, Cres, out, mirror, bn);
}

template <bool TRANS_W, bool EV>
int launch_ws(int nt, int wgs, size_t lds, hipStream_t stream, const float* feat, const float* W, const float* bias, const int32_t* nbr, int n_rows,
              int K, int Cred, int Cres, float* out, int mirror, const BnFuse& bn) {
  if (nt == 1) return apply_launch<conv_apply_ws<1, TRANS_W, EV>>("conv_apply_ws", wgs, WS_WAVES * 64, lds, stream, feat, W, bias, nbr, n_rows, K, Cred, Cres, out, mirror, bn);
  return apply_launch<conv_apply_ws<2, TRANS_W, EV>>("conv_apply_ws", wgs, WS_WAVES * 64, lds, stream, feat, W, bias, nbr, n_rows, K, Cred, Cres, out, mirror, bn);
}

template <bool TRANS_W>
int launch_apply(const float* feat, const float* W, const float* bias, const int32_t* nbr, int n_rows, int K, int Cred,
                 int Cres, float* out, hipStream_t stream, bool bf = false, const int32_t* order = nullptr, int mirror = 0,
                 const BnFuse* bn_ = nullptr) {
  const BnFuse bn = bn_ ? *bn_ : btc_bn_fuse_none();
  if (n_rows <= 0) return BTC_OK;
  BTC_CHECK_ARG(!bf || btc_apply_glds_supported(K, Cred, Cres),
                "bf16 activations need channel counts that are multiples of 16 (K=%d, %d -> %d): convert to fp32", K, Cred, Cres);
  int nt = Cres <= 16 ? 1 : (Cres <= 32 ? 2 : (Cres <= 64 ? 4 : 8));
  const int t_kernel = btc_tune_get(BTC_TUNE_APPLY_KERNEL), t_nt = btc_tune_get(BTC_TUNE_APPLY_NT);
  if (bf || (t_kernel != 1 && btc_apply_glds_supported(K, Cred, Cres) && (t_kernel == 2 || n_rows < 100000 || (Cred >= 64 && Cres >= 64)))) {
    int shape, kc = (Cred % 64 == 0) ? 64 : ((Cred % 32 == 0) ? 32 : 16);
    if (bf) {
      if (Cres % 128 == 0) shape = 424;
      else if (Cres % 64 == 0) shape = n_rows < 8192 ? 141 : 422;
      else if (Cres % 32 == 0) shape = 221;
      else shape = 411;
    } else if (Cres % 128 == 0) {
      shape = n_rows < 7000 ? 222 : (n_rows < 13000 ? 242 : (n_rows <= 16384 ? 424 : (n_rows < 19500 ? 242 : 424)));
    } else if (Cres % 64 == 0) {
      if (kc == 64) shape = n_rows < 11000 ? 141 : 241;
      else shape = n_rows < 13000 ? 141 : 222;
    } else if (Cres % 32 == 0) {
      shape = 221;
    } else {
      shape = 411;
    }
    if (t_nt > 8 && !bf) {
      int wc = (t_nt / 10) % 10, ntw = t_nt % 10;
      while (ntw > 1 && Cres % (16 * wc * ntw)) ntw >>= 1;
      while (wc > 1 && Cres % (16 * wc * ntw)) wc >>= 1;
      const int cand = (t_nt / 100) * 100 + wc * 10 + ntw;
      if (btc_apply_glds_has_shape(cand)) shape = cand;
    }
    const int t_kc = btc_tune_get(BTC_TUNE_APPLY_KC);
    if (t_kc && Cred % t_kc == 0) kc = t_kc;
    while (kc > 16 && btc_apply_glds_lds_bytes(shape, kc, K, bf) > 160 * 1024) kc >>= 1;
    return btc_launch_apply_glds(TRANS_W, shape, kc, apply_flags(mirror), bf, feat, W, bias, nbr, order, n_rows, K, Cred, Cres, out, stream, &bn);
  }
  if (t_kernel != 1 && Cred <= 4 * WS_Q && Cres <= 32 && K <= 64 && n_rows >= 2048 && ws_lds_bytes(K, Cred, nt) <= 160 * 1024) {
    const int n_tiles16 = btc_cdiv(n_rows, 16);
    int wgs = btc_cdiv(n_tiles16, WS_WAVES);
    if (wgs > 256) wgs = 256;
    size_t lds = ws_lds_bytes(K, Cred, nt);
    if (bn.slots && lds < 16 + (size_t)16 * WS_WAVES * 64) lds = 16 + (size_t)16 * WS_WAVES * 64;
    if constexpr (!TRANS_W) {
      if (bn.ev_mean) return launch_ws<false, true>(nt, wgs, lds, stream, feat, W, bias, nbr, n_rows, K, Cred, Cres, out, mirror, bn);
    }
    return launch_ws<TRANS_W, false>(nt, wgs, lds, stream, feat, W, bias, nbr, n_rows, K, Cred, Cres, out, mirror, bn);
  }
  const int tm = 64;
  const int n_tiles = btc_cdiv(n_rows, tm);
  while (nt > 2 && (long long)n_tiles * btc_cdiv(Cres, nt * 16) < 512) nt >>= 1;
  if (t_nt && t_nt <= 8) nt = t_nt;
  dim3 grid(n_tiles, btc_cdiv(Cres, nt * 16));
  size_t lds = (size_t)(tm * LDA + KC * ldb_of(nt)) * sizeof(float) + (size_t)(tm * K + K + 1) * sizeof(int32_t);
  const bool vec = (Cred & 3) == 0;
#define BTC_APPLY(NT_) launch_apply_t<NT_, TRANS_W, 256>(grid, lds, stream, vec, feat, W, bias, nbr, n_rows, K, Cred, Cres, out, mirror, bn)
  switch (nt) {
    case 1: return BTC_APPLY(1);
    case 2: return BTC_APPLY(2);
    case 4: return BTC_APPLY(4);
    default: return BTC_APPLY(8);
  }
#undef BTC_APPLY
}

int split_source_ok(const char* who, long long src_rows, int Cred) {
  BTC_CHECK_ARG(src_rows >= 0, "%s: BTC_OPERANDS_F32_SPLIT needs the row count of src (btc_conv_apply_src / btc_conv_bn_relu_fwd_src)", who);
  BTC_CHECK_ARG(src_rows * Cred * 4 < 0xFFFFFF00LL, "%s: a source of %lld rows x %d channels is past the 32-bit gather offsets of the split-operand "
                "kernel (4 GB): use BTC_OPERANDS_F32", who, src_rows, Cred);
  return BTC_OK;
}

}

int btc_apply(const char* who, int pass, int operands, const void* src, long long src_rows, const void* W, const float* bias, const int32_t* nbr,
              const int32_t* order, int n_rows, int K, int Cin, int Cout, void* dst, hipStream_t stream, const BnFuse* bn) {
  BTC_CHECK_ARG((pass == BTC_PASS_FWD || pass == BTC_PASS_DGRAD || pass == BTC_PASS_DGRAD_MIRROR) && operands >= BTC_OPERANDS_F32 &&
                    operands <= BTC_OPERANDS_F32_SPLIT, "%s: pass=%d operands=%d", who, pass, operands);
  const int mirror = pass == BTC_PASS_DGRAD_MIRROR;
  const bool fwd = pass == BTC_PASS_FWD;
  BTC_CHECK_ARG(K <= BTC_CONV_K_MAX, "%s: K=%d offsets, more than BTC_CONV_K_MAX = %d", who, K, BTC_CONV_K_MAX);
  BTC_CHECK_ARG(K >= 1 && Cin >= 1 && Cout >= 1 && n_rows >= 0, "%s: bad sizes", who);
  BTC_CHECK_ARG(fwd || bias == nullptr, "%s: dgrad takes no bias", who);
  BTC_CHECK_ARG(!bn || Cout <= BN_FUSE_CMAX, "%s: more than %d channels", who, BN_FUSE_CMAX);
  const int Cred = fwd ? Cin : Cout, Cres = fwd ? Cout : Cin;
  if (operands == BTC_OPERANDS_BF16) {
    const bool ok = btc_conv_bf16w_supported(K, Cred, Cres);
    if (bn) BTC_CHECK_ARG(ok, "%s: bf16 operands need K <= 64, Cin %% 32 == 0, Cout %% 16 == 0", who);
    else BTC_CHECK_ARG(ok, "%s: bf16 operands need K <= 64, Cred %% 32 == 0, Cres %% 16 == 0 (K=%d, %d -> %d)", who, K, Cin, Cout);
    return btc_apply_bf16w(src, W, bias, nbr, order, n_rows, K, Cred, Cres, dst, stream, mirror, bn);
  }
  if (operands == BTC_OPERANDS_F32_SPLIT) {
    if (n_rows > 0) {
      const int rc = split_source_ok(who, src_rows, Cred);
      if (rc) return rc;
    }
    return btc_apply_split((const float*)src, W, bias, nbr, order, n_rows, K, Cred, Cres, (float*)dst, stream, mirror, bn);
  }
  const bool bf = operands == BTC_OPERANDS_BF16_ACT;
  if (fwd) return launch_apply<false>((const float*)src, (const float*)W, bias, nbr, n_rows, K, Cred, Cres, (float*)dst, stream, bf, order, 0, bn);
  return launch_apply<true>((const float*)src, (const float*)W, nullptr, nbr, n_rows, K, Cred, Cres, (float*)dst, stream, bf, order, mirror, bn);
}

#define BTC_SIZES_OK(who, n) BTC_CHECK_ARG(K >= 1 && Cin >= 1 && Cout >= 1 && (n) >= 0, who ": bad sizes")

extern "C" int btc_conv_fwd(const float* feat, const float* W, const float* bias, const int32_t* nbr_out, int n_out, int K,
                            int Cin, int Cout, float* out, void* stream) {
  BTC_SIZES_OK("btc_conv_fwd", n_out);
  return btc_apply("btc_conv_fwd", BTC_PASS_FWD, BTC_OPERANDS_F32, feat, -1LL, W, bias, nbr_out, nullptr, n_out, K, Cin, Cout, out, (hipStream_t)stream, nullptr);
}

extern "C" int btc_conv_dgrad(const float* dout, const float* W, const int32_t* nbr_in, int n_in, int K, int Cin, int Cout,
                              float* din, void* stream) {
  BTC_SIZES_OK("btc_conv_dgrad", n_in);
  return btc_apply("btc_conv_dgrad", BTC_PASS_DGRAD, BTC_OPERANDS_F32, dout, -1LL, W, nullptr, nbr_in, nullptr, n_in, K, Cin, Cout, din, (hipStream_t)stream, nullptr);
}

extern "C" int btc_conv_fwd_bf16(const void* feat, const float* W, const float* bias, const int32_t* nbr_out, int n_out, int K,
                                 int Cin, int Cout, void* out, void* stream) {
  BTC_SIZES_OK("btc_conv_fwd_bf16", n_out);
  if (n_out == 0) return BTC_OK;
  return btc_apply("btc_conv_fwd_bf16", BTC_PASS_FWD, BTC_OPERANDS_BF16_ACT, feat, -1LL, W, bias, nbr_out, nullptr, n_out, K, Cin, Cout, out, (hipStream_t)stream, nullptr);
}

extern "C" int btc_conv_dgrad_bf16(const void* dout, const float* W, const int32_t* nbr_in, int n_in, int K, int Cin, int Cout,
                                   void* din, void* stream) {
  BTC_SIZES_OK("btc_conv_dgrad_bf16", n_in);
  if (n_in == 0) return BTC_OK;
  return btc_apply("btc_conv_dgrad_bf16", BTC_PASS_DGRAD, BTC_OPERANDS_BF16_ACT, dout, -1LL, W, nullptr, nbr_in, nullptr, n_in, K, Cin, Cout, din, (hipStream_t)stream, nullptr);
}
#undef BTC_SIZES_OK

extern "C" int btc_conv_fwd_bf16w(const void* feat, const void* wt_bf16, const float* bias, const int32_t* nbr_out, int n_out, int K, int Cin,
                                  int Cout, void* out, void* stream) {
  BTC_CHECK_ARG(n_out >= 0 && btc_conv_bf16w_supported(K, Cin, Cout), "btc_conv_fwd_bf16w: needs K <= 64, Cin %% 32 == 0, Cout %% 16 == 0 (K=%d, %d -> %d)",
                K, Cin, Cout);
  if (n_out == 0) return BTC_OK;
  return btc_apply("btc_conv_fwd_bf16w", BTC_PASS_FWD, BTC_OPERANDS_BF16, feat, -1LL, wt_bf16, bias, nbr_out, nullptr, n_out, K, Cin, Cout, out, (hipStream_t)stream, nullptr);
}

extern "C" int btc_conv_dgrad_bf16w(const void* dout, const void* w_bf16, const int32_t* nbr_in, int n_in, int K, int Cin, int Cout, void* din,
                                    void* stream) {
  BTC_CHECK_ARG(n_in >= 0 && btc_conv_bf16w_supported(K, Cout, Cin), "btc_conv_dgrad_bf16w: needs K <= 64, Cout %% 32 == 0, Cin %% 16 == 0 (K=%d, %d -> %d)",
                K, Cin, Cout);
  if (n_in == 0) return BTC_OK;
  return btc_apply("btc_conv_dgrad_bf16w", BTC_PASS_DGRAD, BTC_OPERANDS_BF16, dout, -1LL, w_bf16, nullptr, nbr_in, nullptr, n_in, K, Cin, Cout, din, (hipStream_t)stream, nullptr);
}

extern "C" int btc_conv_apply_ordered(int pass, int operands, const void* src, const void* W, const float* bias, const int32_t* nbr,
                                      const int32_t* order, int n_rows, int K, int Cin, int Cout, void* dst, void* stream) {
  return btc_apply("btc_conv_apply_ordered", pass, operands, src, pass == BTC_PASS_DGRAD_MIRROR ? (long long)n_rows : -1LL, W, bias, nbr, order, n_rows,
                   K, Cin, Cout, dst, (hipStream_t)stream, nullptr);
}

extern "C" int btc_conv_apply_src(int pass, int operands, const void* src, long long src_rows, const void* W, const float* bias, const int32_t* nbr,
                                  const int32_t* order, int n_rows, int K, int Cin, int Cout, void* dst, void* stream) {
  return btc_apply("btc_conv_apply_src", pass, operands, src, src_rows, W, bias, nbr, order, n_rows, K, Cin, Cout, dst, (hipStream_t)stream, nullptr);
}

extern "C" int btc_maxpool_fwd(const float* feat, const int32_t* nbr_out, int n_out, int K, int C, float* out, void* stream) {
  if (n_out <= 0) return BTC_OK;
  maxpool_fwd_k<<<btc_cdiv((long long)n_out * C, 256), 256, 0, (hipStream_t)stream>>>(feat, nbr_out, n_out, K, C, out);
  BTC_LAUNCH_CHECK();
  return BTC_OK;
}

extern "C" int btc_maxpool_bwd(const float* feat, const float* out, const float* dout, const int32_t* nbr_in, int n_in, int K,
                               int C, float* din, void* stream) {
  if (n_in <= 0) return BTC_OK;
  maxpool_bwd_k<<<btc_cdiv((long long)n_in * C, 256), 256, 0, (hipStream_t)stream>>>(feat, out, dout, nbr_in, n_in, K, C, din);
  BTC_LAUNCH_CHECK();
  return BTC_OK;
}

extern "C" int btc_dense_fwd(const float* feat, const int32_t* indices, int n, int C, const int32_t* h_shape, float* dense,
                             void* stream) {
  if (n <= 0) return BTC_OK;
  dense_fwd_k<<<btc_cdiv((long long)n * C, 256), 256, 0, (hipStream_t)stream>>>(feat, (const int4*)indices, n, C, h_shape[0],
                                                                               h_shape[1], h_shape[2], dense);
  BTC_LAUNCH_CHECK();
  return BTC_OK;
}

extern "C" int btc_dense_bwd(const float* ddense, const int32_t* indices, int n, int C, const int32_t* h_shape, float* dfeat,
                             void* stream) {
  if (n <= 0) return BTC_OK;
  dense_bwd_k<<<btc_cdiv((long long)n * C, 256), 256, 0, (hipStream_t)stream>>>(ddense, (const int4*)indices, n, C, h_shape[0],
                                                                               h_shape[1], h_shape[2], dfeat);
  BTC_LAUNCH_CHECK();
  return BTC_OK;
}
```

include/btcdet_hip.h:

```cpp
#ifndef BTCDET_HIP_H
#define BTCDET_HIP_H

#include <stddef.h>
#include <stdint.h>

#ifdef __cplusplus
extern "C" {
#endif

#define BTC_OK 0
#define BTC_EINVAL (-1)
#define BTC_ELAUNCH (-2)
#define BTC_ERANGE (-3)

#define BTC_MODE_SUBM 0
#define BTC_MODE_CONV 1
#define BTC_MODE_TRANSPOSE 2

const char* btc_last_error(void);
int btc_version(void);

#define BTC_TUNE_APPLY_KERNEL 0
#define BTC_TUNE_APPLY_NT 1
#define BTC_TUNE_APPLY_XCD 2
#define BTC_TUNE_APPLY_KC 4
#define BTC_TUNE_WGRAD_PH 5
#define BTC_TUNE_WGRAD_WGS 6
#define BTC_TUNE_POV_SELECT 7
#define BTC_TUNE_BF16_OPERANDS 8
#define BTC_TUNE_BN_FWD_KB 9
#define BTC_TUNE_BN_BWD_KB 10
#define BTC_TUNE_WGRAD_PIPE 11
#define BTC_TUNE_BN_FUSE 12
#define BTC_TUNE_SPLIT_Z 15
#define BTC_TUNE_SPLIT_LOADERS 17
#define BTC_TUNE_SPLIT 14
#define BTC_TUNE_APPLY_STAGES 13
#define BTC_TUNE_WGRAD_X 18
#define BTC_TUNE_WGRAD_X_DEPTH 20
#define BTC_TUNE_RB_MARK_MULTI 19
#define BTC_TUNE_SPLIT_PAIR 21
#define BTC_TUNE_WGRAD_NARROW 22
#define BTC_TUNE_EVAL_FOLD 23
#define BTC_TUNE_APPLY_DEBUG 3
int btc_tune_set(int key, int value);
int btc_tune_value(int key);

size_t btc_voxelize_ws_bytes(int n, int batch, int max_points);
int btc_voxelize(const float* points, int n, int ld, int xyz_col, int feat_col, int C,
                 const int32_t* scene_offsets, int batch, const float* h_range, const float* h_vsize,
                 const int32_t* h_grid, int max_points, int max_voxels, float* voxels, int32_t* coords,
                 int32_t* num, int32_t* d_total, void* ws, size_t ws_bytes, void* stream);

int btc_cart_to_occ_coords(const float* in, float* out, int n, int ld, int mode, void* stream);

int btc_voxel_shift_col(float* voxels, const int32_t* coords, int m, int max_points, int C, int col,
                        const float* rot_by_batch, float sign, void* stream);

size_t btc_range_mask_ws_bytes(int n);
int btc_range_mask_compact(const float* points, const float* points_b, int n, int ld, int ld_b, const int32_t* scene_offsets, int batch,
                           const float* h_range_xyxy, float* out, float* out_b, int32_t* out_offsets, int32_t* keep_idx, void* ws,
                           size_t ws_bytes, void* stream);
int btc_gather_rows(const float* src, const int32_t* idx, int n_out, int ld, int n_src, float* out, int32_t* bad_count, void* stream);

int btc_out_shape(const int32_t* h_in_shape, const int32_t* h_k, const int32_t* h_s, const int32_t* h_p,
                  const int32_t* h_d, const int32_t* h_outpad, int mode, int32_t* h_out_shape);

size_t btc_rulebook_subm_ws_bytes(int n);
int btc_rulebook_subm(const int32_t* indices, int n, int batch, const int32_t* h_shape, const int32_t* h_k,
                      const int32_t* h_d, int32_t* nbr_out, int32_t* nbr_in, void* ws, size_t ws_bytes,
                      void* stream);

size_t btc_rulebook_conv_ws_bytes(int batch, const int32_t* h_out_shape);
int btc_rulebook_conv_count(const int32_t* indices, int n, int batch, const int32_t* h_in_shape,
                            const int32_t* h_out_shape, const int32_t* h_k, const int32_t* h_s,
                            const int32_t* h_p, const int32_t* h_d, int mode, int32_t* d_n_out, void* ws,
                            size_t ws_bytes, void* stream);
int btc_rulebook_conv_fill(const int32_t* indices, int n, int batch, const int32_t* h_in_shape,
                           const int32_t* h_out_shape, const int32_t* h_k, const int32_t* h_s,
                           const int32_t* h_p, const int32_t* h_d, int mode, int n_out, int32_t* out_indices,
                           int32_t* nbr_out, int32_t* nbr_in, void* ws, size_t ws_bytes, void* stream);

#define BTC_CHAIN_MAX_LAYERS 32
typedef struct BtcChainLayer {
  int32_t kind, ref, mode;
  int32_t in_shape[3], out_shape[3], k[3], s[3], p[3], d[3];
} BtcChainLayer;
size_t btc_chain_ws_bytes(const BtcChainLayer* h_layers, int n_layers, int batch, int n0);
int btc_chain_caps(const BtcChainLayer* h_layers, int n_layers, int batch, int n0, int64_t* h_cap);
int btc_chain_levels(const int32_t* indices, int n0, int batch, const BtcChainLayer* h_layers, int n_layers,
                     int32_t* const* h_out_indices, const int64_t* h_cap, int32_t* d_counts, void* ws, size_t ws_bytes, void* stream);
int btc_chain_maps(const int32_t* indices, int n0, int batch, const BtcChainLayer* h_layers, int n_layers, const int32_t* h_counts,
                   int32_t* const* h_out_indices, int32_t* const* h_nbr_out, int32_t* const* h_nbr_in,
                   int32_t* const* h_first_out ,
                   int32_t* const* h_first_in , void* ws, size_t ws_bytes, void* stream);

size_t btc_pairs_from_nbr_ws_bytes(int n_out, int K);
int btc_pairs_from_nbr(const int32_t* nbr_out, int n_out, int K, int n_in, int32_t* pairs, int32_t* pair_num, void* ws,
                       size_t ws_bytes, void* stream);

int btc_conv_fwd(const float* feat, const float* W, const float* bias , const int32_t* nbr_out,
                 int n_out, int K, int Cin, int Cout, float* out, void* stream);
int btc_conv_dgrad(const float* dout, const float* W, const int32_t* nbr_in, int n_in, int K, int Cin,
                   int Cout, float* din, void* stream);
size_t btc_conv_wgrad_ws_bytes(int n_out, int K, int Cin, int Cout, int n_in);
int btc_conv_wgrad(const float* feat, const float* dout, const int32_t* nbr_out, int n_out, const int32_t* nbr_in,
                   int n_in, int K, int Cin, int Cout, float* dW, void* ws, size_t ws_bytes, void* stream);

int btc_conv_fwd_bf16(const void* feat, const float* W, const float* bias, const int32_t* nbr_out, int n_out, int K, int Cin,
                      int Cout, void* out, void* stream);
int btc_conv_dgrad_bf16(const void* dout, const float* W, const int32_t* nbr_in, int n_in, int K, int Cin, int Cout,
                        void* din, void* stream);
int btc_conv_wgrad_bf16(const void* feat, const void* dout, const int32_t* nbr_out, int n_out, const int32_t* nbr_in,
                        int n_in, int K, int Cin, int Cout, float* dW, void* ws, size_t ws_bytes, void* stream);

int btc_conv_bf16w_supported(int K, int Cred, int Cres);
int btc_weights_to_bf16(const float* W, int K, int Cin, int Cout, void* w_bf16, void* wt_bf16, void* stream);
int btc_weights_to_bf16_multi(const float* const* W, void* const* w_bf16, void* const* wt_bf16, const int32_t* K, const int32_t* Cin,
                              const int32_t* Cout, int n, void* stream);
int btc_conv_fwd_bf16w(const void* feat, const void* wt_bf16, const float* bias, const int32_t* nbr_out, int n_out, int K, int Cin,
                       int Cout, void* out, void* stream);
int btc_conv_dgrad_bf16w(const void* dout, const void* w_bf16, const int32_t* nbr_in, int n_in, int K, int Cin, int Cout, void* din,
                         void* stream);

int btc_conv_split_supported(int K, int Cred, int Cres);
int btc_set_scratch(void* stream, void* ptr, size_t bytes);
int btc_conv_split_wanted(int K, int Cred, int Cres, int n_rows);
int btc_weights_split3(const float* W, int K, int Cin, int Cout, void* w_split, void* wt_split, void* stream);
int btc_weights_split3_multi(const float* const* W, void* const* w_split, void* const* wt_split, const int32_t* K, const int32_t* Cin,
                             const int32_t* Cout, int n, void* stream);

#define BTC_ROW_ORDER_MAX_MAPS 64
#define BTC_PASS_FWD 0
#define BTC_PASS_DGRAD 1
#define BTC_PASS_DGRAD_MIRROR 2
#define BTC_OPERANDS_F32 0
#define BTC_OPERANDS_BF16_ACT 1
#define BTC_OPERANDS_BF16 2
#define BTC_OPERANDS_F32_SPLIT 3
#define BTC_CONV_K_MAX 512
int btc_row_orders(const int32_t* const* nbrs , const int32_t* n_rows ,
                   const int32_t* Ks , int n_maps, int32_t* order , void* stream);
int btc_row_orders_keyed(const int32_t* const* nbrs, const int32_t* const* firsts, const int32_t* n_rows, const int32_t* Ks, int n_maps,
                         int32_t* order, void* stream);
int btc_conv_apply_ordered(int pass, int operands, const void* src, const void* W, const float* bias, const int32_t* nbr,
                           const int32_t* order, int n_rows, int K, int Cin, int Cout, void* dst, void* stream);
int btc_conv_apply_src(int pass, int operands, const void* src, long long src_rows, const void* W, const float* bias, const int32_t* nbr,
                       const int32_t* order, int n_rows, int K, int Cin, int Cout, void* dst, void* stream);
int btc_conv_wgrad_ordered(int bf16_act, const void* feat, const void* dout, const int32_t* nbr_out, int n_out,
                           const int32_t* nbr_in, int n_in, const int32_t* order_out, const int32_t* order_in, int K, int Cin,
                           int Cout, float* dW, void* ws, size_t ws_bytes, void* stream);
#define BTC_WGRAD_MULTI_MAX 64
int btc_conv_wgrad_slabs(int bf16_act, const void* feat, const void* dout, const int32_t* nbr_out, int n_out, const int32_t* nbr_in,
                         int n_in, const int32_t* order_out, const int32_t* order_in, int K, int Cin, int Cout, float* dW, void* ws,
                         size_t ws_bytes, int* n_slabs, void* stream);
int btc_wgrad_reduce_multi(const float* const* parts, float* const* dWs, const int* n_slabs, const long long* counts, int n_jobs,
                           void* stream);


#define BTC_ADAM_MAX_SEGMENTS 448
int btc_adam_max_segments(void);
size_t btc_adam_group_ws_bytes(int n_chunks);
int btc_grads_pack(const float* const* grads, int n_seg, const int32_t* chunk_seg, const int32_t* chunk_off,
                   const int32_t* chunk_len, const int64_t* chunk_flat, const int32_t* seg_chunk0, float* flat, void* stream);
int btc_adam_group_step(const float* const* grads, int n_seg, const int32_t* chunk_seg, const int32_t* chunk_off,
                        const int32_t* chunk_len, const int64_t* chunk_flat, const int32_t* seg_chunk0, int n_chunks,
                        float* params, float* exp_avg, float* exp_avg_sq, long long step, float lr, float beta1, float beta2,
                        float eps, float weight_decay, float clip, void* ws, size_t ws_bytes, void* stream);

int btc_maxpool_fwd(const float* feat, const int32_t* nbr_out, int n_out, int K, int C, float* out, void* stream);
int btc_maxpool_bwd(const float* feat, const float* out, const float* dout, const int32_t* nbr_in, int n_in,
                    int K, int C, float* din, void* stream);

int btc_dense_fwd(const float* feat, const int32_t* indices, int n, int C, const int32_t* h_shape, float* dense,
                  void* stream);
int btc_dense_bwd(const float* ddense, const int32_t* indices, int n, int C, const int32_t* h_shape, float* dfeat,
                  void* stream);
int btc_dense_split_fwd(const float* feat, const int32_t* indices, int n, int Ca, int Cb, const int32_t* h_shape, float* dense_a,
                        float* dense_b, void* stream);
int btc_dense_split_bwd(const float* grad_a, const float* grad_b, const int32_t* indices, int n, int Ca, int Cb,
                        const int32_t* h_shape, float* dfeat, void* stream);
int btc_occ_prob(const float* logit, const unsigned char* mask, int B, long long ncell, float* prob, void* stream);
int btc_cat_pad_fwd(const void* a, int ca, const void* b, int cb, long long n, int cout, int elem_bytes, void* out, void* stream);
int btc_cat_pad_bwd(const void* grad, int cout, long long n, int elem_bytes, void* da, int ca, void* db, int cb, void* stream);
int btc_spin(int microseconds, void* stream);
size_t btc_sumsq2_ws_bytes(void);
int btc_sumsq2_fwd(const void* a, long long na, int a_bf16, double ka, const void* b, long long nb, int b_bf16, double kb, float* out,
                   void* ws, size_t ws_bytes, void* stream);
int btc_sumsq2_bwd(const void* a, long long na, int a_bf16, float ka2, void* da, const void* b, long long nb, int b_bf16, float kb2,
                   void* db, const float* g, void* stream);


size_t btc_revoxelize_ws_bytes(int n, int batch, const int32_t* h_shape);
int btc_revoxelize_count(const int64_t* coords, int n, int batch, const int32_t* h_shape, int32_t* d_m,
                         int32_t* d_pmax, void* ws, size_t ws_bytes, void* stream);
int btc_revoxelize_fill(const float* points, const int64_t* coords, int n, int C, int batch,
                        const int32_t* h_shape, int m, int pmax, float* voxels, int64_t* vcoords,
                        int64_t* vnum, void* ws, size_t ws_bytes, void* stream);

typedef struct BtcOccConfig {
  int32_t batch;
  int32_t grid[3];
  int32_t sphere_grid[3];
  int32_t dist_kern[3];
  int32_t concede_x;
  int32_t empt_sur_thresh;
  int32_t max_boxes;
  int32_t use_box_weight;
  float occ_range[6], occ_voxel[3];
  float sphere_range[6], sphere_voxel[3];
  float det_zmin, det_zmax;
  float w_fore_cls, w_mirr_cls, w_bm_cls, w_neg_cls, w_fore_res, w_mirr_res, w_bm_res, box_weight;
  const int32_t* backproject_lut;
  int32_t reverse_vis;
  int32_t vis_half;
} BtcOccConfig;

typedef struct BtcOccBuffers {
  uint8_t *vcc_mask, *voxelwise_mask, *bm_voxelwise_mask, *occ_voxelwise_mask, *fore_voxelwise_mask, *pos_mask,
      *general_cls_loss_mask, *occ_fore_cls_mask, *occ_mirr_cls_mask, *occ_bm_cls_mask, *general_reg_loss_mask;
  int8_t* forebox_label;
  float *general_cls_loss_mask_float, *general_reg_loss_mask_float, *res_mtrx;
  int32_t* pos_all_num;
} BtcOccBuffers;

size_t btc_occ_targets_ws_bytes(const BtcOccConfig* cfg);
int btc_occ_backproject_lut(const BtcOccConfig* cfg, int32_t* lut, void* stream);
int btc_occ_targets(const BtcOccConfig* cfg, float* voxels, const int32_t* voxel_coords, const int32_t* voxel_num,
                    int M, int max_points, int C, const float* gt_boxes, const int32_t* gt_num, const float* mirr_flag,
                    const float* bm_points, int n_bm, const float* rot_z, const float* centers,
                    const BtcOccBuffers* out, void* ws, size_t ws_bytes, void* stream);

size_t btc_bn_ws_bytes(int C);
int btc_bn_relu_fwd(const float* x, int N, int C, const float* gamma, const float* beta, float* running_mean,
                    float* running_var, long long* num_batches_tracked, float momentum, float eps, int training,
                    int relu, float* y, float* save_mean, float* save_rstd, void* ws, size_t ws_bytes, void* stream);
int btc_bn_relu_bwd(const float* x, const float* y, const float* dy, int N, int C, const float* gamma,
                    const float* save_mean, const float* save_rstd, int training, int relu, float* dx, float* dgamma,
                    float* dbeta, void* ws, size_t ws_bytes, void* stream);
int btc_bn_relu_fwd_bf16(const void* x, int N, int C, const float* gamma, const float* beta, float* running_mean,
                         float* running_var, long long* num_batches_tracked, float momentum, float eps, int training,
                         int relu, void* y, float* save_mean, float* save_rstd, void* ws, size_t ws_bytes, void* stream);
int btc_bn_relu_bwd_bf16(const void* x, const void* y, const void* dy, int N, int C, const float* gamma,
                         const float* save_mean, const float* save_rstd, int training, int relu, void* dx, float* dgamma,
                         float* dbeta, void* ws, size_t ws_bytes, void* stream);
size_t btc_bn_fuse_ws_bytes(void);
int btc_conv_bn_relu_fwd(int operands, const void* src, const void* W, const float* bias, const int32_t* nbr, const int32_t* order,
                         int n_rows, int K, int Cin, int Cout, void* x, const float* gamma, const float* beta, float* running_mean,
                         float* running_var, long long* num_batches_tracked, float momentum, float eps, int relu, void* y,
                         float* save_mean, float* save_rstd, void* ws, size_t ws_bytes, void* fuse_ws, void* stream);
int btc_conv_bn_relu_fwd_src(int operands, const void* src, long long src_rows, const void* W, const float* bias, const int32_t* nbr, const int32_t* order,
                         int n_rows, int K, int Cin, int Cout, void* x, const float* gamma, const float* beta, float* running_mean,
                         float* running_var, long long* num_batches_tracked, float momentum, float eps, int relu, void* y,
                         float* save_mean, float* save_rstd, void* ws, size_t ws_bytes, void* fuse_ws, void* stream);
int btc_col_sum(const float* x, int N, int C, float* out, void* ws, size_t ws_bytes, void* stream);
int btc_col_sum_bf16(const void* x, int N, int C, float* out, void* ws, size_t ws_bytes, void* stream);

typedef struct BtcPovConfig {
  int32_t batch, max_k;
  int32_t occ_grid[3];
  int32_t det_grid[3];
  float occ_origin[3], occ_voxel[3];
  float det_origin[3], det_voxel[3];
  float occ_thresh, inten;
  int32_t code_dim;
} BtcPovConfig;

size_t btc_pass_occ_vox_ws_bytes(const BtcPovConfig* cfg, int M, int P);
int btc_pass_occ_vox_count(const BtcPovConfig* cfg, const float* probs , const float* residuals ,
                           const uint8_t* use_occ , const float* rot_z , const int32_t* det_coords,
                           const int32_t* det_num, int M, int P, int C, int32_t* d_info, void* ws, size_t ws_bytes, void* stream);
int btc_pass_occ_vox_fill(const BtcPovConfig* cfg, const float* det_voxels, int M, int P, int C, int m, int pmax, int k_total,
                          float* voxels, int64_t* vcoords, int64_t* vnum, float* occ_pnts, int64_t* occ_b, void* ws,
                          size_t ws_bytes, void* stream);
int btc_pass_occ_vox_fill_i32(const BtcPovConfig* cfg, const float* det_voxels, int M, int P, int C, int m, int pmax, int k_total,
                              float* voxels, int64_t* vcoords, int64_t* vnum, float* occ_pnts, int64_t* occ_b, int32_t* vcoords32,
                              int32_t* vnum32, void* ws, size_t ws_bytes, void* stream);

size_t btc_occ_loss_ws_bytes(void);
int btc_occ_loss_fwd(const float* logit, const float* res, const float* res_target, const uint8_t* pos_mask,
                     const uint8_t* cls_mask, const float* cls_w, const uint8_t* reg_mask, const float* reg_w, int B,
                     long long ncell, float beta, float w_cls, float w_res, float* out2, float* norms2, void* ws, size_t ws_bytes,
                     void* stream);
int btc_occ_loss_bwd(const float* logit, const float* res, const float* res_target, const uint8_t* pos_mask,
                     const uint8_t* cls_mask, const float* cls_w, const uint8_t* reg_mask, const float* reg_w, int B,
                     long long ncell, float beta, const float* norms2, const float* grad2, float* d_logit, float* d_res, void* stream);
int btc_occ_loss_fwd_total(const float* logit, const float* res, const float* res_target, const uint8_t* pos_mask,
                           const uint8_t* cls_mask, const float* cls_w, const uint8_t* reg_mask, const float* reg_w, int B,
                           long long ncell, float beta, float w_cls, float w_res, float* out3, float* norms2, void* ws, size_t ws_bytes,
                           void* stream);
int btc_occ_loss_bwd_total(const float* logit, const float* res, const float* res_target, const uint8_t* pos_mask,
                           const uint8_t* cls_mask, const float* cls_w, const uint8_t* reg_mask, const float* reg_w, int B,
                           long long ncell, float beta, const float* norms2, const float* grad_total, float* d_logit, float* d_res,
                           void* stream);

int btc_mean_vfe(const float* voxels, const void* num_points, int num_is_float, int M, int P, int C, float* out, void* stream);
int btc_occ_vfe(const float* voxels, const void* num_points, int num_is_float, int M, int P, int F, int R, float* feat,
                float* occ, void* stream);

int btc_boxes_pairwise_bev(const float* boxes_a, int na, const float* boxes_b, int nb, int mode, float* out, void* stream);
size_t btc_nms_ws_bytes(int n);
int btc_nms(const float* boxes_sorted, int n, float thresh, int rotated, long long* keep, int32_t* d_num_keep, void* ws,
            size_t ws_bytes, void* stream);
int btc_trilinear_corners(const float* xyz, long long n_points, long long points_per_batch, const float* range_lo, const float* voxel,
                          const float* stride_zyx, const int32_t* grid_dhw, int batch, const int32_t* cell_row, const uint8_t* row_live,
                          int32_t* rows, float* weights, uint8_t* flag, void* stream);
int btc_trilinear_gather(const float* feat, int C, long long n_keep, const int32_t* rows, const float* weights, float* out, void* stream);
int btc_trilinear_scatter(const float* grad_out, int C, const int32_t* pair_sorted, const int32_t* seg, const float* weights, int n_rows,
                          float* grad_feat, void* stream);

size_t btc_nms_topk_ws_bytes(int batch, int n, int max_keep);
int btc_nms_topk(const float* boxes_sorted, int batch, int n, float thresh, int rotated, int max_keep, long long* keep,
                 int32_t* num_keep, void* ws, size_t ws_bytes, void* stream);


int btc_ball_query(const float* new_xyz, const int32_t* new_xyz_batch_cnt, const float* xyz, const int32_t* xyz_batch_cnt, int B,
                   int M, float inner_radius, float outer_radius, int nsample, int32_t* idx, void* stream);
int btc_group_points(const float* features, const int32_t* features_batch_cnt, const int32_t* idx, const int32_t* idx_batch_cnt,
                     int B, int M, int C, int nsample, float* out, void* stream);
int btc_group_points_grad(const float* grad_out, const int32_t* idx, const int32_t* idx_batch_cnt, const int32_t* features_batch_cnt,
                          int B, int M, int C, int N, int nsample, float* grad_features, void* stream);
int btc_furthest_point_sampling(const float* xyz, int B, int N, int npoint, float* temp, int32_t* idx, void* stream);
int btc_three_nn(const float* unknown, const int32_t* unknown_batch_cnt, const float* known, const int32_t* known_batch_cnt, int B,
                 int N, float* dist2, int32_t* idx, void* stream);
int btc_three_interpolate(const float* features, const int32_t* idx, const float* weight, int N, int C, float* out, void* stream);
int btc_three_interpolate_grad(const float* grad_out, const int32_t* idx, const float* weight, int N, int C, int M,
                               float* grad_features, void* stream);

#ifdef __cplusplus
}
#endif
#endif
```

Baseline: 591.3.

## Pack multiple kernel offsets per reduction chunk in gather-GEMM for narrow channels

For narrow-channel layers (Cred 16 or 32), the glds apply kernel now packs 2 or 4 kernel offsets into one KC-wide reduction item. Each pipeline stage gathers rows from several neighbours and the matching weight slices, so narrow layers need fewer, fuller pipeline iterations. The gather path also switches from flat-pointer global-to-LDS loads to buffer-resource loads, where an out-of-range offset replaces the explicit zero-row pointer, whenever the source fits in the descriptor range. This adds template instances and per-offset activity masking, and a shape heuristic chooses the pack factor.

New measurement: 585.7. About the same (-1.0%).

```diff
diff --git a/btcdet_amd/csrc/btc_common.h b/btcdet_amd/csrc/btc_common.h
--- a/btcdet_amd/csrc/btc_common.h
+++ b/btcdet_amd/csrc/btc_common.h
@@ -56,17 +56,18 @@
 
 bool btc_apply_glds_supported(int K, int Cred, int Cres);
 bool btc_apply_glds_has_shape(int shape, bool bf = false);
+bool btc_apply_glds_has_pack(int shape, bool bf);
 size_t btc_apply_glds_lds_bytes(int shape, int kc, int K, bool bf, int stages = 3);
 int btc_apply_glds_stages(int shape, int kc, int K, bool bf, int asked);
-int btc_launch_apply_glds(bool trans_w, int shape, int kc, int xcd, bool bf, const void* feat, const float* W, const float* bias,
+int btc_launch_apply_glds(bool trans_w, int shape, int kc, int pk, int xcd, bool bf, const void* feat, const float* W, const float* bias,
                           const int32_t* nbr, const int32_t* order , int n_rows, int K, int Cred, int Cres, void* out,
                           hipStream_t stream, const struct BnFuse* bn = nullptr );
 
 int btc_apply(const char* who, int pass, int operands, const void* src, long long src_rows, const void* W, const float* bias, const int32_t* nbr,
               const int32_t* order, int n_rows, int K, int Cin, int Cout, void* dst, hipStream_t stream, const struct BnFuse* bn);
 
-int btc_apply_bf16w(const void* src, const void* Wq, const float* bias, const int32_t* nbr, const int32_t* order, int n_rows, int K, int Cred,
-                    int Cres, void* dst, hipStream_t stream, int mirror = 0, const struct BnFuse* bn = nullptr);
+int btc_apply_bf16w(const void* src, long long src_rows, const void* Wq, const float* bias, const int32_t* nbr, const int32_t* order, int n_rows, int K,
+                    int Cred, int Cres, void* dst, hipStream_t stream, int mirror = 0, const struct BnFuse* bn = nullptr);
 constexpr size_t BTC_SCRATCH_HEAD = 64 * 1024;
 constexpr long long BTC_SCRATCH_TICKETS = BTC_SCRATCH_HEAD / 4;
 void* btc_scratch(hipStream_t stream, size_t* bytes);
diff --git a/btcdet_amd/csrc/conv_apply_bf16.hip b/btcdet_amd/csrc/conv_apply_bf16.hip
--- a/btcdet_amd/csrc/conv_apply_bf16.hip
+++ b/btcdet_amd/csrc/conv_apply_bf16.hip
@@ -40,6 +40,8 @@
   for (int nt = 0; nt < NTW; ++nt) acc[nt] = (f32x4){0.f, 0.f, 0.f, 0.f};
 
   int iq = 0, ir = 0, cq = 0, cr = 0;
+  const bool by_ptr = flags & APPLY_PTR;
+  const __amdgpu_buffer_rsrc_t rfeat = __builtin_amdgcn_make_buffer_rsrc((void*)feat, 0, BTC_RSRC_RECORDS, 0x00020000);
   auto issue = [&](int st) {
     const int k = s_kact[PAIR ? 2 * iq : iq];
     const int k1 = (PAIR && 2 * iq + 1 < n_act) ? s_kact[2 * iq + 1] : -1;
@@ -56,8 +58,9 @@
         const int u = (U % UPR) ^ ((rloc / RPB) & (UPR - 1));
         const int ku = (PAIR && (u & 4)) ? k1 : k;
         const int nb = ku >= 0 ? s_nbr[rloc * K + ku] : -1;
-        const unsigned short* src = nb >= 0 ? feat + (size_t)nb * Cred + cc + (PAIR ? (u & 3) : u) * 8 : g_zero_row_b;
-        glds16(src, As + ai * 1024);
+        const unsigned col = (unsigned)(cc + (PAIR ? (u & 3) : u) * 8);
+        if (by_ptr) glds16(nb >= 0 ? feat + (size_t)nb * Cred + col : g_zero_row_b, As + ai * 1024);
+        else blds16s(rfeat, nb >= 0 ? ((unsigned)nb * (unsigned)Cred + col) * 2u : BTC_RSRC_ABSENT, As + ai * 1024);
       }
     }
     const unsigned short* Wk = Wq + ((size_t)k * Cres + n0) * Cred + cc;
@@ -148,7 +151,7 @@
   return launch_b<WR, WC, NTW, 32>(feat, Wq, bias, nbr, order, n_rows, K, Cred, Cres, out, xcd, stream, bn);
 }
 
-int apply_b(const void* feat_, const void* Wq_, const float* bias, const int32_t* nbr, const int32_t* order, int n_rows, int K, int Cred, int Cres,
+int apply_b(const void* feat_, long long src_rows, const void* Wq_, const float* bias, const int32_t* nbr, const int32_t* order, int n_rows, int K, int Cred, int Cres,
             void* out_, hipStream_t stream, int mirror = 0, const BnFuse* bn_ = nullptr) {
   if (n_rows <= 0) return BTC_OK;
   const BnFuse bn = bn_ ? *bn_ : btc_bn_fuse_none();
@@ -157,7 +160,7 @@
   unsigned short* out = (unsigned short*)out_;
   int kc = (Cred % 64 == 0) ? 64 : 32;
   if (Cred == 32 && K >= 8 && btc_tune_get(BTC_TUNE_SPLIT_PAIR) != 1 && (btc_tune_get(BTC_TUNE_SPLIT_PAIR) == 2 || n_rows >= 5000)) kc = 128;
-  const int xcd = apply_flags(mirror);
+  const int xcd = apply_flags(mirror) | (apply_desc_reaches(src_rows, Cred, 2) ? 0 : APPLY_PTR);
   if (Cres % 128 == 0) return launch_b_kc<4, 2, 4>(kc, feat, Wq, bias, nbr, order, n_rows, K, Cred, Cres, out, xcd, stream, bn);
   if (Cres % 64 == 0) {
     if (n_rows < 8192) return launch_b_kc<1, 4, 1>(kc, feat, Wq, bias, nbr, order, n_rows, K, Cred, Cres, out, xcd, stream, bn);
@@ -216,9 +219,9 @@
   return BTC_OK;
 }
 
-int btc_apply_bf16w(const void* src, const void* Wq, const float* bias, const int32_t* nbr, const int32_t* order, int n_rows, int K, int Cred,
-                    int Cres, void* dst, hipStream_t stream, int mirror, const BnFuse* bn) {
-  return apply_b(src, Wq, bias, nbr, order, n_rows, K, Cred, Cres, dst, stream, mirror, bn);
+int btc_apply_bf16w(const void* src, long long src_rows, const void* Wq, const float* bias, const int32_t* nbr, const int32_t* order, int n_rows, int K,
+                    int Cred, int Cres, void* dst, hipStream_t stream, int mirror, const BnFuse* bn) {
+  return apply_b(src, src_rows, Wq, bias, nbr, order, n_rows, K, Cred, Cres, dst, stream, mirror, bn);
 }
 
 extern "C" int btc_conv_bf16w_supported(int K, int Cred, int Cres) { return K >= 1 && K <= 64 && Cred >= 32 && Cred % 32 == 0 && Cres % 16 == 0; }
diff --git a/btcdet_amd/csrc/conv_apply_glds.hip b/btcdet_amd/csrc/conv_apply_glds.hip
--- a/btcdet_amd/csrc/conv_apply_glds.hip
+++ b/btcdet_amd/csrc/conv_apply_glds.hip
@@ -20,7 +20,7 @@
   y0 = __uint_as_float(x0); y1 = __uint_as_float(x1); y2 = __uint_as_float(x2); y3 = __uint_as_float(x3);
 }
 
-template <int WR, int WC, int NTW, bool TRANS_W, int KC, bool BF>
+template <int WR, int WC, int NTW, bool TRANS_W, int KC, bool BF, int PK = 1>
 __global__ __launch_bounds__(64 * WR * WC) void conv_apply_g(const void* __restrict__ feat_, const float* __restrict__ W,
                                                              const float* __restrict__ bias, const int32_t* __restrict__ nbr,
                                                              const int32_t* __restrict__ order, int n_rows, int K, int Cred, int Cres,
@@ -50,8 +50,11 @@
   const ApplyTile tile = apply_tile_prologue<TM, THREADS>(s_nbr, s_kact, s_nact, s_row, nbr, order, n_rows, K, flags, wr);
   const int bx = tile.bx, n0 = blockIdx.y * TN, n_act = tile.n_act;
   const unsigned long long wave_act = tile.wave_act;
-  const int n_chunks = Cred / KC;
-  const int n_items = (dbg & 32) ? 0 : n_act * n_chunks;
+  static_assert(PK == 1 || ((PK == 2 || PK == 4) && KC / PK >= 16), "PK offsets of a KC / PK-channel reduction per item");
+  constexpr int CO = KC / PK;
+  constexpr int UO = UPR / PK;
+  const int n_chunks = PK > 1 ? 1 : Cred / KC;
+  const int n_items = (dbg & 32) ? 0 : (PK > 1 ? (n_act + PK - 1) / PK : n_act * n_chunks);
   if (dbg & 16) return;
 
   f32x4 acc[NTW];
@@ -59,8 +62,12 @@
   for (int nt = 0; nt < NTW; ++nt) acc[nt] = (f32x4){0.f, 0.f, 0.f, 0.f};
 
   int iq = 0, ir = 0, cq = 0, cr = 0;
+  const bool by_ptr = flags & APPLY_PTR;
+  const __amdgpu_buffer_rsrc_t rfeat = __builtin_amdgcn_make_buffer_rsrc((void*)feat_, 0, BTC_RSRC_RECORDS, 0x00020000);
+  const unsigned row_bytes = (unsigned)Cred * ES;
   auto issue = [&](int st) {
-    const int k = s_kact[iq];
+    const int q0 = PK * iq;
+    const int k = s_kact[q0];
     const int cc = ir * KC;
     if (++ir == n_chunks) { ir = 0; ++iq; }
     char* As = ring + st * STAGE;
@@ -73,9 +80,18 @@
       if (A_UNITS % 64 == 0 || U < A_UNITS) {
         const int rloc = U / UPR;
         const int u = (U % UPR) ^ ((rloc / RPB) & (UPR - 1));
-        const int nb = s_nbr[rloc * K + k];
-        const char* src = nb >= 0 ? feat + ((size_t)nb * Cred + cc) * ES + u * 16 : (const char*)g_zero_row;
-        glds16(src, As + ai * 1024);
+        int nb;
+        unsigned off;
+        if (PK == 1) {
+          nb = s_nbr[rloc * K + k];
+          off = (unsigned)(cc * ES + u * 16);
+        } else {
+          const int j = u / UO;
+          nb = q0 + j < n_act ? s_nbr[rloc * K + s_kact[q0 + j]] : -1;
+          off = (unsigned)((u % UO) * 16);
+        }
+        if (by_ptr) glds16(nb >= 0 ? feat + (size_t)nb * row_bytes + off : (const char*)g_zero_row, As + ai * 1024);
+        else blds16s(rfeat, nb >= 0 ? (unsigned)nb * row_bytes + off : BTC_RSRC_ABSENT, As + ai * 1024);
       }
     }
     const float* Wk = W + (size_t)k * Cred * Cres;
@@ -88,11 +104,23 @@
       if (!TRANS_W) {
         const int kr = U / (TN / 4), pu = U % (TN / 4);
         const int g = (NG >= 2) ? ((pu >> 2) ^ (kr & 1)) : (pu >> 2);
-        src = Wk + (size_t)(cc + kr) * Cres + n0 + g * 16 + (pu & 3) * 4;
+        if (PK == 1) {
+          src = Wk + (size_t)(cc + kr) * Cres + n0 + g * 16 + (pu & 3) * 4;
+        } else {
+          const int j = kr / CO;
+          const int kj = q0 + j < n_act ? s_kact[q0 + j] : k;
+          src = W + ((size_t)kj * Cred + kr % CO) * Cres + n0 + g * 16 + (pu & 3) * 4;
+        }
       } else {
         const int c = U / UPB, pu = U % UPB;
         const int ru = pu ^ (c & (UPB - 1));
-        src = Wk + (size_t)(n0 + c) * Cred + cc + ru * 4;
+        if (PK == 1) {
+          src = Wk + (size_t)(n0 + c) * Cred + cc + ru * 4;
+        } else {
+          const int j = ru / (CO / 4);
+          const int kj = q0 + j < n_act ? s_kact[q0 + j] : k;
+          src = W + ((size_t)kj * Cres + n0 + c) * Cred + (ru % (CO / 4)) * 4;
+        }
       }
       glds16(src, Bs + ii * 256);
     }
@@ -117,9 +145,15 @@
     __builtin_amdgcn_s_barrier();
     asm volatile("" ::: "memory");
     if (item + S - 1 < n_items && !(dbg & 2)) issue(st == 0 ? S - 1 : st - 1);
-    const int k = s_kact[cq];
+    bool act[PK], any = false;
+#pragma unroll
+    for (int j = 0; j < PK; ++j) {
+      const int k = PK * cq + j < n_act ? s_kact[PK * cq + j] : -1;
+      act[j] = k >= 0 && ((wave_act >> (k & 63)) & 1ull);
+      any |= act[j];
+    }
     if (++cr == n_chunks) { cr = 0; ++cq; }
-    if (((wave_act >> k) & 1ull) && !(dbg & 1)) {
+    if (any && !(dbg & 1)) {
       const char* A = ring + st * STAGE + (wr * 16 + arow) * (KC * ES);
       const float* B = (const float*)(ring + st * STAGE + A_BYTES);
       const int aswz = ((wr * 16 + arow) / RPB) & (UPR - 1);
@@ -180,10 +214,12 @@
         if (g + 1 < NGRP) load_group(g + 1, (g + 1) & 1);
         __builtin_amdgcn_sched_barrier(0);
 #pragma unroll
-        for (int i = 0; i < G; ++i)
+        for (int i = 0; i < G; ++i) {
+          if (PK > 1 && !act[(g * G + i) / (Q / PK)]) continue;
 #pragma unroll
           for (int nt = 0; nt < NTW; ++nt)
             acc[nt] = __builtin_amdgcn_mfma_f32_16x16x4f32(a[g & 1][i], b[g & 1][i][nt], acc[nt], 0, 0, 0);
+        }
         __builtin_amdgcn_sched_barrier(0);
       }
     }
@@ -204,14 +240,14 @@
   }
 }
 
-template <int WR, int WC, int NTW, bool TRANS_W, int KC, bool BF>
+template <int WR, int WC, int NTW, bool TRANS_W, int KC, bool BF, int PK = 1>
 int launch_g(const void* feat, const float* W, const float* bias, const int32_t* nbr, const int32_t* order, int n_rows, int K, int Cred,
              int Cres, void* out, int xcd, hipStream_t stream, const BnFuse& bn) {
   constexpr int TM = 16 * WR, TN = 16 * NTW * WC;
   const int stages = btc_apply_glds_stages(WR * 100 + WC * 10 + NTW, KC, K, BF, (xcd >> APPLY_STAGES_SHIFT) & 15);
-  xcd = (xcd & (APPLY_XCD | APPLY_MIRROR)) | (stages << APPLY_STAGES_SHIFT);
+  xcd = (xcd & (APPLY_XCD | APPLY_MIRROR | APPLY_PTR)) | (stages << APPLY_STAGES_SHIFT);
   const size_t lds = btc_apply_glds_lds_bytes(WR * 100 + WC * 10 + NTW, KC, K, BF, stages);
-  return apply_launch<conv_apply_g<WR, WC, NTW, TRANS_W, KC, BF>>("conv_apply_g", dim3(btc_cdiv(n_rows, TM), Cres / TN), 64 * WR * WC, lds, stream, feat, W,
+  return apply_launch<conv_apply_g<WR, WC, NTW, TRANS_W, KC, BF, PK>>("conv_apply_g", dim3(btc_cdiv(n_rows, TM), Cres / TN), 64 * WR * WC, lds, stream, feat, W,
                                                                   bias, nbr, order, n_rows, K, Cred, Cres, out, xcd,
                                                                   btc_tune_get(BTC_TUNE_APPLY_DEBUG), bn);
 }
@@ -230,9 +266,28 @@
   }
 }
 
+template <int WR, int WC, int NTW, bool TRANS_W, bool BF>
+int launch_g_pk(int kc, int pk, G_PARAMS) {
+  if (kc == 32) return launch_g<WR, WC, NTW, TRANS_W, 32, BF, 2>(G_ARGS);
+  if (pk == 2) return launch_g<WR, WC, NTW, TRANS_W, 64, BF, 2>(G_ARGS);
+  return launch_g<WR, WC, NTW, TRANS_W, 64, BF, 4>(G_ARGS);
+}
+
 template <bool TRANS_W>
-int launch_g_shape(int wr, int wc, int ntw, int kc, bool bf, G_PARAMS) {
+int launch_g_shape(int wr, int wc, int ntw, int kc, int pk, bool bf, G_PARAMS) {
   const int code = wr * 100 + wc * 10 + ntw;
+  if (pk > 1) {
+    switch (code) {
+#define G_PACK2(WR_, WC_, NTW_)                                                      \
+  case WR_ * 100 + WC_ * 10 + NTW_:                                                  \
+    return bf ? launch_g_pk<WR_, WC_, NTW_, TRANS_W, true>(kc, pk, G_ARGS) : launch_g_pk<WR_, WC_, NTW_, TRANS_W, false>(kc, pk, G_ARGS)
+      G_PACK2(4, 1, 1); G_PACK2(2, 2, 1); G_PACK2(1, 4, 1);
+#undef G_PACK2
+      default: break;
+    }
+    btc_set_error("conv_apply_g: no packed instance for WR=%d WC=%d NTW=%d bf16=%d", wr, wc, ntw, (int)bf);
+    return BTC_EINVAL;
+  }
   switch (code) {
 #define G_CASE2(WR_, WC_, NTW_)                                                      \
   case WR_ * 100 + WC_ * 10 + NTW_:                                                  \
@@ -269,6 +324,8 @@
   return false;
 }
 
+bool btc_apply_glds_has_pack(int shape, bool) { return shape == 411 || shape == 221 || shape == 141; }
+
 size_t btc_apply_glds_lds_bytes(int shape, int kc, int K, bool bf, int stages) {
   const int tm = 16 * (shape / 100), tn = 16 * ((shape / 10) % 10) * (shape % 10);
   const size_t a_bytes = ((size_t)tm * kc * (bf ? 2 : 4) + 1023) / 1024 * 1024;
@@ -292,14 +349,15 @@
 
 bool btc_apply_glds_supported(int K, int Cred, int Cres) { return K <= 64 && Cred % 16 == 0 && Cres % 16 == 0 && Cred >= 16; }
 
-int btc_launch_apply_glds(bool trans_w, int shape, int kc, int xcd, bool bf, const void* feat, const float* W, const float* bias,
+int btc_launch_apply_glds(bool trans_w, int shape, int kc, int pk, int xcd, bool bf, const void* feat, const float* W, const float* bias,
                           const int32_t* nbr, const int32_t* order, int n_rows, int K, int Cred, int Cres, void* out, hipStream_t stream,
                           const BnFuse* bn_) {
   if (n_rows <= 0) return BTC_OK;
   const BnFuse bn = bn_ ? *bn_ : btc_bn_fuse_none();
   const int wr = shape / 100, wc = (shape / 10) % 10, ntw = shape % 10;
-  BTC_CHECK_ARG(btc_apply_glds_supported(K, Cred, Cres) && wc * ntw > 0 && Cres % (16 * wc * ntw) == 0 && Cred % kc == 0 &&
-                    (kc == 16 || kc == 32 || kc == 64),
-                "conv_apply_g: unsupported K=%d Cred=%d Cres=%d shape=%d kc=%d", K, Cred, Cres, shape, kc);
-  return trans_w ? launch_g_shape<true>(wr, wc, ntw, kc, bf, G_ARGS) : launch_g_shape<false>(wr, wc, ntw, kc, bf, G_ARGS);
-}
+  BTC_CHECK_ARG(btc_apply_glds_supported(K, Cred, Cres) && wc * ntw > 0 && Cres % (16 * wc * ntw) == 0 && (pk > 1 || Cred % kc == 0) &&
+                    (kc == 16 || kc == 32 || kc == 64) &&
+                    (pk == 1 || ((pk == 2 || pk == 4) && kc == pk * Cred && btc_apply_glds_has_pack(shape, bf))),
+                "conv_apply_g: unsupported K=%d Cred=%d Cres=%d shape=%d kc=%d pk=%d", K, Cred, Cres, shape, kc, pk);
+  return trans_w ? launch_g_shape<true>(wr, wc, ntw, kc, pk, bf, G_ARGS) : launch_g_shape<false>(wr, wc, ntw, kc, pk, bf, G_ARGS);
+}
diff --git a/btcdet_amd/csrc/conv_apply_split.hip b/btcdet_amd/csrc/conv_apply_split.hip
--- a/btcdet_amd/csrc/conv_apply_split.hip
+++ b/btcdet_amd/csrc/conv_apply_split.hip
@@ -2,11 +2,6 @@
 
 namespace {
 
-#define BTC_RSRC_RECORDS 0xFFFFFF00u
-#define BTC_RSRC_ABSENT 0xFFFFFFF0u
-__device__ __forceinline__ void blds16s(__amdgpu_buffer_rsrc_t rsrc, unsigned voffset, void* l) {
-  __builtin_amdgcn_raw_ptr_buffer_load_lds(rsrc, (__attribute__((address_space(3))) void*)l, 16, voffset, 0, 0, 0);
-}
 
 template <int WR, int WC, int NTW, int KC, int S_STAGES, int LW, bool PAIR = false>
 __global__ __launch_bounds__(64 * (WR * WC + LW)) void conv_apply_s(const float* __restrict__ feat, const unsigned short* __restrict__ Ws,
diff --git a/btcdet_amd/csrc/conv_tile.h b/btcdet_amd/csrc/conv_tile.h
--- a/btcdet_amd/csrc/conv_tile.h
+++ b/btcdet_amd/csrc/conv_tile.h
@@ -8,6 +8,7 @@
 
 constexpr int APPLY_XCD = 1;
 constexpr int APPLY_MIRROR = 2;
+constexpr int APPLY_PTR = 4;
 constexpr int APPLY_STAGES_SHIFT = 4;
 constexpr int APPLY_DEBUG_SHIFT = 8;
 inline int apply_flags(int mirror) { return (btc_tune_get(BTC_TUNE_APPLY_XCD) == 2 ? APPLY_XCD : 0) | (mirror ? APPLY_MIRROR : 0); }
@@ -99,6 +100,12 @@
 __device__ __forceinline__ void wait_vm() {
   asm volatile("s_waitcnt vmcnt(%0)" ::"n"(N) : "memory");
 }
+#define BTC_RSRC_RECORDS 0xFFFFFF00u
+#define BTC_RSRC_ABSENT 0xFFFFFFF0u
+__device__ __forceinline__ void blds16s(__amdgpu_buffer_rsrc_t rsrc, unsigned voffset, void* l) {
+  __builtin_amdgcn_raw_ptr_buffer_load_lds(rsrc, (__attribute__((address_space(3))) void*)l, 16, voffset, 0, 0, 0);
+}
+inline bool apply_desc_reaches(long long src_rows, int C, int es) { return src_rows >= 0 && src_rows * C * es < (long long)BTC_RSRC_RECORDS; }
 
 __device__ __forceinline__ float btc_split_rest(float x) { return x - __uint_as_float(__float_as_uint(x) & 0xFFFF0000u); }
 struct BtcSplit3 { unsigned hi, mid, lo; };
diff --git a/btcdet_amd/csrc/sparse_conv.hip b/btcdet_amd/csrc/sparse_conv.hip
--- a/btcdet_amd/csrc/sparse_conv.hip
+++ b/btcdet_amd/csrc/sparse_conv.hip
@@ -359,8 +359,14 @@
   return apply_launch<conv_apply_ws<2, TRANS_W, EV>>("conv_apply_ws", wgs, WS_WAVES * 64, lds, stream, feat, W, bias, nbr, n_rows, K, Cred, Cres, out, mirror, bn);
 }
 
+int apply_pack_wanted(bool bf, int shape, int Cred, int n_rows) {
+  if (bf) return 1;
+  if (Cred == 16) return (shape == 221 || shape == 411) ? 2 : 1;
+  return (shape == 221 && n_rows < 60000) ? 2 : 1;
+}
+
 template <bool TRANS_W>
-int launch_apply(const float* feat, const float* W, const float* bias, const int32_t* nbr, int n_rows, int K, int Cred,
+int launch_apply(const float* feat, long long src_rows, const float* W, const float* bias, const int32_t* nbr, int n_rows, int K, int Cred,
                  int Cres, float* out, hipStream_t stream, bool bf = false, const int32_t* order = nullptr, int mirror = 0,
                  const BnFuse* bn_ = nullptr) {
   const BnFuse bn = bn_ ? *bn_ : btc_bn_fuse_none();
@@ -396,7 +402,16 @@
     const int t_kc = btc_tune_get(BTC_TUNE_APPLY_KC);
     if (t_kc && Cred % t_kc == 0) kc = t_kc;
     while (kc > 16 && btc_apply_glds_lds_bytes(shape, kc, K, bf) > 160 * 1024) kc >>= 1;
-    return btc_launch_apply_glds(TRANS_W, shape, kc, apply_flags(mirror), bf, feat, W, bias, nbr, order, n_rows, K, Cred, Cres, out, stream, &bn);
+    int pk = 1;
+    const int t_pack = btc_tune_get(BTC_TUNE_APPLY_PACK);
+    if (t_pack != 1 && (Cred == 16 || Cred == 32) && btc_apply_glds_has_pack(shape, bf)) {
+      pk = t_pack == 2 ? ((t_kc == 32 && Cred == 16) ? 2 : 64 / Cred) : apply_pack_wanted(bf, shape, Cred, n_rows);
+      if (pk > 1 && btc_apply_glds_lds_bytes(shape, pk * Cred, K, bf) > 160 * 1024) pk = 1;
+      if (pk > 1) kc = pk * Cred;
+    }
+    int flags = apply_flags(mirror) | (apply_desc_reaches(src_rows, Cred, bf ? 2 : 4) ? 0 : APPLY_PTR);
+    if (pk > 1 && t_pack == 0 && !btc_tune_get(BTC_TUNE_APPLY_STAGES)) flags |= 3 << APPLY_STAGES_SHIFT;
+    return btc_launch_apply_glds(TRANS_W, shape, kc, pk, flags, bf, feat, W, bias, nbr, order, n_rows, K, Cred, Cres, out, stream, &bn);
   }
   if (t_kernel != 1 && Cred <= 4 * WS_Q && Cres <= 32 && K <= 64 && n_rows >= 2048 && ws_lds_bytes(K, Cred, nt) <= 160 * 1024) {
     const int n_tiles16 = btc_cdiv(n_rows, 16);
@@ -450,7 +465,7 @@
     const bool ok = btc_conv_bf16w_supported(K, Cred, Cres);
     if (bn) BTC_CHECK_ARG(ok, "%s: bf16 operands need K <= 64, Cin %% 32 == 0, Cout %% 16 == 0", who);
     else BTC_CHECK_ARG(ok, "%s: bf16 operands need K <= 64, Cred %% 32 == 0, Cres %% 16 == 0 (K=%d, %d -> %d)", who, K, Cin, Cout);
-    return btc_apply_bf16w(src, W, bias, nbr, order, n_rows, K, Cred, Cres, dst, stream, mirror, bn);
+    return btc_apply_bf16w(src, src_rows, W, bias, nbr, order, n_rows, K, Cred, Cres, dst, stream, mirror, bn);
   }
   if (operands == BTC_OPERANDS_F32_SPLIT) {
     if (n_rows > 0) {
@@ -460,8 +475,8 @@
     return btc_apply_split((const float*)src, W, bias, nbr, order, n_rows, K, Cred, Cres, (float*)dst, stream, mirror, bn);
   }
   const bool bf = operands == BTC_OPERANDS_BF16_ACT;
-  if (fwd) return launch_apply<false>((const float*)src, (const float*)W, bias, nbr, n_rows, K, Cred, Cres, (float*)dst, stream, bf, order, 0, bn);
-  return launch_apply<true>((const float*)src, (const float*)W, nullptr, nbr, n_rows, K, Cred, Cres, (float*)dst, stream, bf, order, mirror, bn);
+  if (fwd) return launch_apply<false>((const float*)src, src_rows, (const float*)W, bias, nbr, n_rows, K, Cred, Cres, (float*)dst, stream, bf, order, 0, bn);
+  return launch_apply<true>((const float*)src, src_rows, (const float*)W, nullptr, nbr, n_rows, K, Cred, Cres, (float*)dst, stream, bf, order, mirror, bn);
 }
 
 #define BTC_SIZES_OK(who, n) BTC_CHECK_ARG(K >= 1 && Cin >= 1 && Cout >= 1 && (n) >= 0, who ": bad sizes")
diff --git a/include/btcdet_hip.h b/include/btcdet_hip.h
--- a/include/btcdet_hip.h
+++ b/include/btcdet_hip.h
@@ -37,6 +37,7 @@
 #define BTC_TUNE_SPLIT 14
 #define BTC_TUNE_APPLY_STAGES 13
 #define BTC_TUNE_WGRAD_X 18
+#define BTC_TUNE_APPLY_PACK 16
 #define BTC_TUNE_WGRAD_X_DEPTH 20
 #define BTC_TUNE_RB_MARK_MULTI 19
 #define BTC_TUNE_SPLIT_PAIR 21
```
